# Linyou/Ced-NeRF

Measured on AMD Instinct MI355X. Metric: samples_per_sec (render_image_test, 800x800 D-NeRF lego-shaped synthetic), higher is better.
Workload: dtype f32 (MLP GEMMs: split-fp16 MFMA, 22-bit operands, fp32 accumulate)

## Files before the change

ced_nerf_amd/_lib.py:

```python
from __future__ import annotations

import ctypes as C
import os
import subprocess
from typing import List, Optional

_PKG = os.path.dirname(os.path.abspath(__file__))
_ROOT = os.path.dirname(_PKG)
LIB_PATH = os.environ.get("CED_NERF_LIB", os.path.join(_PKG, "libcednerf_hip.so"))
SOURCES = ["runtime.hip", "march.hip", "composite.hip", "field.hip", "field_half.hip", "field_mixed.hip", "field_move.hip", "field_jacobian.hip", "frame.hip", "occgrid.hip",
           "raygen.hip", "wgrad.hip", "pixels.hip", "accel.hip", "linear.hip", "mlp.hip", "train_glue.hip", "losses.hip",
           "metrics.hip", "train_batch.hip", "importance.hip", "bake.hip", "mesh.hip"]
MLP_F32, MLP_F16X2, MLP_F16, MLP_F32_HEAD16X2 = 0, 1, 2, 3
MLP_PRECISIONS = {"f32": MLP_F32, "f16x2": MLP_F16X2, "f16": MLP_F16, "f32+h16x2": MLP_F32_HEAD16X2}
HIPCC_FLAGS = ["--offload-arch=gfx950", "-O3", "-ffp-contract=off", "-fno-slp-vectorize", "-fPIC", "-shared", "-std=c++17"]
PER_SOURCE_FLAGS = {"field_half.hip": ["-mllvm", "-amdgpu-sched-strategy=max-memory-clause"]}
MAX_LEVELS = 16


class HashDesc(C.Structure):
    _fields_ = [
        ("n_levels", C.c_int32), ("table_dtype", C.c_int32), ("temporal", C.c_int32), ("reserved", C.c_int32),
        ("scale", C.c_float * MAX_LEVELS), ("res", C.c_uint32 * MAX_LEVELS), ("offset", C.c_uint32 * MAX_LEVELS),
        ("size", C.c_uint32 * MAX_LEVELS), ("hashed", C.c_uint32 * MAX_LEVELS),
        ("table", C.c_void_p), ("total_entries", C.c_uint64),
    ]


class FieldDesc(C.Structure):
    _fields_ = [
        ("aabb", C.c_float * 6), ("moving_step", C.c_float), ("use_div_offsets", C.c_int32),
        ("time_mode", C.c_int32), ("mlp_precision", C.c_int32), ("max_workgroups", C.c_int32),
        ("packed_weights", C.c_void_p), ("packed_floats", C.c_uint64),
        ("hash", HashDesc),
    ]


class FrameTrace(C.Structure):
    _fields_ = [
        ("capacity", C.c_int32), ("n_iters", C.c_int32),
        ("field_begin", C.POINTER(C.c_void_p)), ("field_end", C.POINTER(C.c_void_p)),
        ("iter_alive", C.POINTER(C.c_int64)), ("iter_n_samples", C.POINTER(C.c_int64)),
        ("iter_samples", C.POINTER(C.c_int64)), ("field_stamps", C.c_void_p),
    ]


EXCHANGE_FN = C.CFUNCTYPE(C.c_int, C.c_void_p, C.c_void_p, C.c_int32, C.c_int32, C.c_void_p)


class ShardExchange(C.Structure):
    _fields_ = [
        ("global_rays_per_frame", C.c_int64), ("local_rays", C.c_void_p), ("counts", C.c_void_p),
        ("reduce", EXCHANGE_FN), ("user", C.c_void_p),
    ]


_vp, _i64, _i32, _f = C.c_void_p, C.c_int64, C.c_int32, C.c_float

PROTOTYPES = {
    "ced_version": (C.c_int, []),
    "ced_last_error_string": (C.c_char_p, []),
    "ced_set_option": (C.c_int, [C.c_char_p, C.c_int]),
    "ced_packed_weight_floats": (_i64, [C.c_int, C.c_int]),
    "ced_pack_field_weights": (C.c_int, [C.c_int, C.c_int] + [_vp] * 10),
    "ced_packed_weight_words": (_i64, [C.c_int, C.c_int, C.c_int]),
    "ced_pack_field_weights_half": (C.c_int, [C.c_int, C.c_int, C.c_int] + [_vp] * 10),
    "ced_pack_field_weights_half_for": (C.c_int, [C.c_int] * 5 + [_vp] * 10),
    "ced_pack_field_weights_mixed": (C.c_int, [C.c_int, C.c_int] + [_vp] * 10),
    "ced_ray_aabb_intersect": (C.c_int, [_i64, _vp, _vp, _i32, _vp, _f, _f, _f, _vp, _vp, _vp, _vp]),
    "ced_sort_intersections": (C.c_int, [_i64, _i32, _vp, _vp, _vp, _vp, _vp]),
    "ced_traverse_grids": (C.c_int, [_i64, _vp, _vp, _vp, _i32, _i32, _vp, _vp, _vp, _f, _f, _i32, _vp, _vp, _vp, _vp,
                                     _i32, _vp, _vp, _vp, _vp, _vp, _vp, _vp, _vp]),
    "ced_host_skip_march": (_f, [_f, _f, _f, _f]),
    "ced_occupancy_accel_bytes": (_i64, [_i32, _i32]),
    "ced_build_occupancy_accel": (C.c_int, [_vp, _i32, _i32, _vp, _i64, _vp]),
    "ced_host_build_occupancy_accel": (C.c_int, [_vp, _i32, _i32, _vp]),
    "ced_host_count_steps": (_i32, [C.POINTER(C.c_float), _f, _f, _i32, C.POINTER(C.c_float)]),
    "ced_host_march_frame": (C.c_int, [_i64, _vp, _vp, _vp, _i32, _i32, _vp, _vp, _f, _f, _f, _i32, _vp, _vp, _vp, _vp, _i32, _i32,
                                       _i32, _vp, _vp, _vp, _vp]),
    "ced_hash_encode": (C.c_int, [C.POINTER(HashDesc), _i64, _vp, _vp, _vp, _vp]),
    "ced_hash_encode_backward": (C.c_int, [C.POINTER(HashDesc), _i64, _vp, _vp, _vp, _vp, _i32, _vp]),
    "ced_hash_encode_backward_temporal": (C.c_int, [C.POINTER(HashDesc), _i64, _vp, _vp, _vp, _vp, _vp]),
    "ced_field_forward": (C.c_int, [C.POINTER(FieldDesc), _i64, _vp, _vp, _vp, _vp, _vp, _vp, _vp]),
    "ced_field_forward_rays": (C.c_int, [C.POINTER(FieldDesc), _i64, _vp, _vp, _vp, _vp, _vp, _vp, _vp, _i32, _i32,
                                         _vp, _vp, _vp]),
    "ced_field_move": (C.c_int, [C.POINTER(FieldDesc), _i64, _vp, _vp, _vp, _vp, _vp, _vp, _vp]),
    "ced_field_move_rays": (C.c_int, [C.POINTER(FieldDesc), _i64, _vp, _vp, _vp, _vp, _vp, _vp, _vp, _i32, _vp, _vp, _vp]),
    "ced_field_move_inverse": (C.c_int, [C.POINTER(FieldDesc), _i64, _vp, _vp, _vp, _i32, _f, _vp, _vp, _vp, _vp]),
    "ced_field_track": (C.c_int, [C.POINTER(FieldDesc), _i64, _i64, _vp, _vp, _vp, _i32, _f, _vp, _vp, _vp, _vp]),
    "ced_field_move_jacobian": (C.c_int, [C.POINTER(FieldDesc), _i64, _vp, _vp, _vp, _vp, _vp]),
    "ced_field_move_inverse_newton": (C.c_int, [C.POINTER(FieldDesc), _i64, _vp, _vp, _vp, _i32, _f, _vp, _vp, _vp, _vp]),
    "ced_field_track_newton": (C.c_int, [C.POINTER(FieldDesc), _i64, _i64, _vp, _vp, _vp, _i32, _f, _vp, _vp, _vp, _vp]),
    "ced_field_rgb": (C.c_int, [C.POINTER(FieldDesc), _i64, _vp, _vp, _i32, _vp, _vp]),
    "ced_field_rgb_bcast": (C.c_int, [C.POINTER(FieldDesc), _i64, _i32, _vp, _vp, _i32, _vp, _vp]),
    "ced_bake_workspace_bytes": (_i64, [_i64]),
    "ced_bake_candidates": (C.c_int, [_i32, C.POINTER(C.c_float), _f, _i64, _i64, _vp, _vp, _i32, _i32, _i64, _vp, _vp, _vp,
                                      _vp, _i64, _vp]),
    "ced_bake_select": (C.c_int, [_i64, _vp, _vp, _vp, _vp, _f, _i64, _vp, _vp, _vp, _vp, _vp, _vp, _i64, _vp]),
    "ced_mesh_workspace_bytes": (_i64, [_i32]),
    "ced_mesh_vertices": (C.c_int, [_i32, C.POINTER(C.c_float), _f, _vp, _f, _i64, _vp, _vp, _vp, _vp, _vp, _i64, _vp]),
    "ced_mesh_faces": (C.c_int, [_i32, _vp, _f, _vp, _i64, _i64, _vp, _vp, _vp, _i64, _vp]),
    "ced_render_weights": (C.c_int, [_i64, _vp, _vp, _vp, _vp, _vp, _vp, _vp, _vp, _vp]),
    "ced_accumulate_along_rays": (C.c_int, [_i64, _vp, _vp, _vp, _i32, _vp, _vp]),
    "ced_reduce_along_rays": (C.c_int, [_i64, _vp, _vp, _i32, _vp, _i32, _i64, _i32, _vp, _vp, _vp]),
    "ced_visibility_mask": (C.c_int, [_i64, _vp, _vp, _vp, _vp, _f, _f, _vp, _vp]),
    "ced_composite_prefix": (C.c_int, [_i64, _vp, _vp, _vp, _vp, _vp, _vp, _vp, _vp, _vp]),
    "ced_composite_backward": (C.c_int, [_i64, _vp, _vp, _vp, _vp, _vp, _vp, _vp, _vp, _vp, _vp, _vp]),
    "ced_distortion_workspace_bytes": (_i64, [_i64, _i64, _i32]),
    "ced_distortion_loss": (C.c_int, [_i64, _i64] + [_vp] * 10),
    "ced_distortion_loss_density": (C.c_int, [_i64, _i64] + [_vp] * 10),
    "ced_ssim_workspace_bytes": (_i64, [_i64, _i64, _i64, _i64, _i32, _i32]),
    "ced_ssim": (C.c_int, [_i64, _i64, _i64, _i64, _vp, C.POINTER(_i64), _vp, C.POINTER(_i64), C.c_double, C.c_double,
                           C.c_double, _i32, C.POINTER(C.c_float), _i32, C.POINTER(C.c_float), _i32, _vp, _vp, _vp, _vp,
                           _vp, _vp]),
    "ced_frame_to_rgb8": (C.c_int, [_i32, _i32, _vp, _i32, _vp, _vp]),
    "ced_depth_to_u8": (C.c_int, [_i32, _i32, _vp, _i32, _vp, _vp, _vp]),
    "ced_scatter_pixels": (C.c_int, [_i64, _vp, _i32, _vp, _i32, _vp, _i32, _vp, _i64, _vp, _vp, _vp, _vp, _i32, _i32, _vp]),
    "ced_linear": (C.c_int, [_i64, _vp, _i32, _vp, _i32, _i32, _i32, _i32, _i32, _vp, _vp, _vp]),
    "ced_weight_grad_workspace_bytes": (_i64, [_i64, _i32, _i32]),
    "ced_weight_grad": (C.c_int, [_i64, _vp, _i32, _vp, _i32, _vp, _vp, _i64, _vp]),
    "ced_composite_step": (C.c_int, [_i64, _vp, _vp, _vp, _vp, _vp, _vp, _vp, _vp, _f, _i32, _vp, _vp, _vp]),
    "ced_composite_test": (C.c_int, [_i64, _vp, _vp, _vp, _vp, _vp, _vp, _f, _f, _vp, _vp, _vp, _vp]),
    "ced_finalize_pixels": (C.c_int, [_i64, _vp, _vp, _vp, _vp, _vp]),
    "ced_occ_cell_points": (C.c_int, [_i64, _vp, _vp, _i32, C.POINTER(C.c_float), _vp, _vp]),
    "ced_occ_ema_update": (C.c_int, [_i64, _vp, _vp, _f, _f, _vp, _vp]),
    "ced_generate_rays_pinhole": (C.c_int, [_i32, _i32, _f, _f, _f, _f, C.POINTER(C.c_float), _i32, _vp, _vp, _vp, _vp]),
    "ced_generate_rays_hypercam": (C.c_int, [_i32, _i32, C.POINTER(C.c_float), C.POINTER(C.c_float), _f, _f, _f, _f, _f,
                                             C.POINTER(C.c_float), C.POINTER(C.c_float), _vp, _vp, _vp]),
    "ced_sample_training_batch": (C.c_int, [_i32] * 5 + [_vp] * 3 + [_i64, C.c_uint64, _i64, _i32, _i32] + [_vp] * 7),
    "ced_importance_batch_workspace_bytes": (_i64, [_i64, _i64, _i64]),
    "ced_sample_importance_batch": (C.c_int, [_i32] * 5 + [_vp] * 4 + [_i32, _i64, _i64, C.c_uint64, _i64, _i32] + [_vp] * 8
                                    + [_i64, _vp]),
    "ced_temporal_median_u8": (C.c_int, [_i32] * 4 + [_vp] * 3),
    "ced_isg_weights": (C.c_int, [_i32] * 4 + [_vp, _vp, _f, _vp, _vp]),
    "ced_ist_weights": (C.c_int, [_i32] * 4 + [_vp, _f, _i32, _vp, _vp]),
    "ced_render_image_test_workspace_bytes": (_i64, [_i64, _i32, _i32, _f, _i32]),
    "ced_render_image_test": (C.c_int, [C.POINTER(FieldDesc), _i64, _vp, _vp, _vp, _i32, _i32, _vp, _vp, _f, _f, _f, _f, _f,
                                        _i32, _vp, _i32, _vp, _vp, _vp, _vp, _vp, _i64, _vp, C.POINTER(_i64),
                                        C.POINTER(FrameTrace), _vp, _vp]),
    "ced_render_frames_test_workspace_bytes": (_i64, [_i32, _i64, _i32, _i32, _f, _i32]),
    "ced_render_frames_test": (C.c_int, [C.POINTER(FieldDesc), _i32, _i64, _vp, _vp, _vp, _i32, _i32, _vp, _vp, _f, _f, _f, _f,
                                         _f, _i32, _vp, _vp, _vp, _vp, _vp, _vp, _i64, _vp, C.POINTER(_i64),
                                         C.POINTER(FrameTrace), _vp, _vp]),
    "ced_render_frames_test_sharded_workspace_bytes": (_i64, [_i32, _i64, _i64, _i32, _i32, _f, _i32]),
    "ced_render_frames_test_iterations": (_i32, [_f, _i32]),
    "ced_render_frames_test_host_bytes": (_i64, [_f, _i32]),
    "ced_render_frames_test_sharded": (C.c_int, [C.POINTER(FieldDesc), _i32, _i64, _vp, _vp, _vp, _i32, _i32, _vp, _vp, _f, _f, _f,
                                                 _f, _f, _i32, _vp, _vp, _vp, _vp, _vp, _vp, _i64, _vp, C.POINTER(_i64),
                                                 C.POINTER(FrameTrace), _vp, _vp, C.POINTER(ShardExchange)]),
    "ced_wall_clock_khz": (_i64, []),
    "ced_mlp_chain": (C.c_int, [_i64, _i32, _i32, _vp, C.POINTER(_i32), C.POINTER(_vp), C.POINTER(_vp), C.POINTER(_vp), _i32, _vp]),
    "ced_march_all": (C.c_int, [_i64, _vp, _vp, _vp, _i32, _i32, _vp, _vp, _vp, _f, _f, _f, _vp, _vp, _vp, _i32, _vp, _vp, _vp,
                                _vp, _i64, _vp, _vp]),
    "ced_render_image_workspace_bytes": (_i64, [_i64, _i64]),
    "ced_render_image": (C.c_int, [C.POINTER(FieldDesc), _i64, _vp, _vp, _i64, _vp, _vp, _vp, _f, _f, _vp, _i32, _vp, _vp, _vp,
                                   _vp, _vp, _vp, _i64, _vp, C.POINTER(_i64), _vp, _vp]),
    "ced_mlp_backward_dw_workspace_bytes": (_i64, [_i64, _i32, C.POINTER(_i32)]),
    "ced_mlp_backward_dw": (C.c_int, [_i64, _i32, _vp, C.POINTER(_i32), C.POINTER(_vp), C.POINTER(_vp), _vp, _vp, _vp, _i64, _vp]),
    "ced_train_inputs": (C.c_int, [_i64] + [_vp] * 13),
    "ced_train_warp": (C.c_int, [_i64, _vp, _vp, _i32, _i32, _f, C.POINTER(C.c_float), _vp, _vp, _vp, _vp]),
    "ced_train_warp_backward": (C.c_int, [_i64, _vp, _vp, _i32, _i32, _f, C.POINTER(C.c_float), _vp, _vp, _vp, _vp]),
    "ced_train_head_in": (C.c_int, [_i64] + [_vp] * 6),
    "ced_train_head_in_backward": (C.c_int, [_i64] + [_vp] * 6),
    "ced_render_image_gather": (C.c_int, [_i64, _i64, _i64, _vp, _i64, _vp, _i64, _vp, _vp, _vp, _vp, _vp, _vp, _vp, _vp, _vp]),
}


def _includes(path: str, seen=None) -> List[str]:
    import re
    seen = set() if seen is None else seen
    if path in seen or not os.path.exists(path):
        return []
    seen.add(path)
    out = [path]
    for inc in re.findall(r'^\s*#\s*include\s+"([^"]+)"', open(path).read(), flags=re.M):
        out += _includes(os.path.normpath(os.path.join(os.path.dirname(path), inc)), seen)
    return out


def build(force: bool = False, verbose: bool = False, extra_flags: Optional[List[str]] = None) -> str:
    from concurrent.futures import ThreadPoolExecutor
    srcs = [os.path.join(_PKG, "csrc", s) for s in SOURCES]
    hipcc = os.environ.get("HIPCC", "hipcc")
    flags = [f for f in HIPCC_FLAGS if f != "-shared"] + list(extra_flags or [])
    obj_dir = os.path.join(_ROOT, "build", "obj")
    os.makedirs(obj_dir, exist_ok=True)
    stamp = os.path.join(obj_dir, "flags.txt")
    flag_text = " ".join([hipcc] + flags + [f"{k}:{' '.join(v)}" for k, v in sorted(PER_SOURCE_FLAGS.items())])
    if not os.path.exists(stamp) or open(stamp).read() != flag_text:
        force = True
    jobs, objs = [], []
    for src in srcs:
        obj = os.path.join(obj_dir, os.path.basename(src) + ".o")
        objs.append(obj)
        deps = _includes(src)
        if force or not os.path.exists(obj) or any(os.path.getmtime(obj) < os.path.getmtime(d) for d in deps):
            jobs.append([hipcc] + flags + PER_SOURCE_FLAGS.get(os.path.basename(src), []) + ["-c", src, "-o", obj])
    if not jobs and os.path.exists(LIB_PATH) and all(os.path.getmtime(LIB_PATH) >= os.path.getmtime(o) for o in objs):
        return LIB_PATH

    def run(cmd):
        if verbose:
            print(" ".join(cmd), flush=True)
        subprocess.check_call(cmd)

    workers = max(1, min(len(jobs), int(os.environ.get("CED_BUILD_JOBS", str(min(os.cpu_count() or 1, 8))))))
    if jobs:
        with ThreadPoolExecutor(max_workers=workers) as pool:
            list(pool.map(run, jobs))
    run([hipcc, "--offload-arch=gfx950", "-shared", "-fPIC", "-o", LIB_PATH] + objs)
    from . import _k32_gate
    _, bad = _k32_gate.check(LIB_PATH)
    if bad:
        os.remove(LIB_PATH)
        raise RuntimeError("K = 32 residency gate failed (ced_nerf_amd/_k32_gate.py): "
                           + "; ".join(f"{k}: {v}" for k, v in sorted(bad.items())))
    with open(stamp, "w") as f:
        f.write(flag_text)
    return LIB_PATH


_lib: Optional[C.CDLL] = None


def lib() -> C.CDLL:
    global _lib
    if _lib is None:
        if not os.path.exists(LIB_PATH):
            raise RuntimeError(
                f"{LIB_PATH} not found: build the HIP extension first (python -c 'import __graft_entry__ as g; "
                "g.build()'); ced_nerf_amd has no CPU fallback")
        handle = C.CDLL(LIB_PATH)
        for name, (res, args) in PROTOTYPES.items():
            fn = getattr(handle, name)
            fn.restype = res
            fn.argtypes = args
        _lib = handle
        for item in filter(None, os.environ.get("CED_OPTIONS", "").split(",")):
# ... 18 lines not shown
```

ced_nerf_amd/csrc/field.hip:

```cpp
#include <atomic>
#include <cstring>

#include "ced_common.hpp"
#include "field_args.hpp"
#include "field_device.hpp"
#include "field_kernel.hpp"

namespace ced {


struct HashArgs {
    int64_t n;
    const float *x, *t;
    float *out;
    int n_levels, table_dtype, temporal;
    const void *table;
    float scale[CED_MAX_LEVELS];
    uint32_t res[CED_MAX_LEVELS], offset[CED_MAX_LEVELS], size[CED_MAX_LEVELS], hashed[CED_MAX_LEVELS];
};

template <bool F16, bool TEMPORAL>
__global__ __launch_bounds__(256) void hash_encode_kernel(HashArgs A)
{
    const int64_t i = (int64_t)blockIdx.x * blockDim.x + threadIdx.x;
// ... 276 lines not shown
    }
    A.level_mode = 0;
    for (int i = 0; i < 4; ++i) {
        int n_hashed = 0;
        bool pairs = !A.temporal;
        for (int g = 0; g < 4; ++g) {
            const int l = 4 * i + g;
            n_hashed += d->hash.hashed[l] ? 1 : 0;
            pairs = pairs && l + 1 < d->hash.n_levels &&
                    (uint64_t)d->hash.offset[l] + d->hash.size[l] < d->hash.total_entries;
        }
        A.level_mode |= (n_hashed == 0 ? (pairs ? 3 : 1) : (n_hashed == 4 ? 2 : 0)) << (2 * i);
    }
    CED_REQUIRE(d->hash.total_entries * (uint64_t)((A.table_dtype ? 4 : 8) * (A.temporal ? 4 : 1)) < (1ull << 32),
                "field_forward: hash table larger than 4 GiB");
    CED_REQUIRE(d->max_workgroups >= 0 && d->max_workgroups <= 65536, "field_forward: max_workgroups=%d", d->max_workgroups);
    A.max_blocks = d->max_workgroups;
    A.spread_tiles = g_field_spread_tiles;
    if (d->mlp_precision == CED_MLP_F32_HEAD16X2) return launch_field_mixed(A, d->time_mode, stream);
    if (d->mlp_precision != CED_MLP_F32) {
        return launch_field_half(A, d->time_mode, d->mlp_precision, stream);
    }
    switch ((d->time_mode ? 1 : 0) | (A.table_dtype ? 2 : 0) | (A.temporal ? 4 : 0)) {
    case 0: launch_field_grid<2, 1024>(field_kernel<false, false, false, 2, 1024>, A, stream); break;
    case 1: launch_field_grid<2, 1024>(field_kernel<true, false, false, 2, 1024>, A, stream); break;
    case 2: launch_field_grid<2, 1024>(field_kernel<false, true, false, 2, 1024>, A, stream); break;
    case 3: launch_field_grid<2, 1024>(field_kernel<true, true, false, 2, 1024>, A, stream); break;
    case 4: launch_field_grid<2, 512>(field_kernel<false, false, true, 2, 512>, A, stream); break;
    case 5: launch_field_grid<2, 512>(field_kernel<true, false, true, 2, 512>, A, stream); break;
    case 6: launch_field_grid<2, 512>(field_kernel<false, true, true, 2, 512>, A, stream); break;
    default: launch_field_grid<2, 512>(field_kernel<true, true, true, 2, 512>, A, stream); break;
    }
    return check_launch("field_forward");
}

}

extern "C" int ced_set_option(const char *key, int value)
{
    CED_REQUIRE(key != nullptr, "set_option: null key");
    if (strcmp(key, "field_spread_tiles") == 0) {
        CED_REQUIRE(value >= 0 && value <= 2, "set_option: field_spread_tiles must be 0, 1 or 2 (field_tile_range)");
        ced::g_field_spread_tiles = value;
        return CED_OK;
    }
    if (strcmp(key, "march_two_pass") == 0) {
        CED_REQUIRE(value >= -1 && value <= 1, "set_option: march_two_pass must be -1 (automatic), 0 or 1");
        ced::g_march_two_pass = value;
        return CED_OK;
    }
    if (strcmp(key, "hash_grad_blocks") == 0) {
        CED_REQUIRE(value >= 0 && value <= (1 << 20), "set_option: hash_grad_blocks must be 0 (no cap) .. 2^20");
        ced::g_hash_grad_blocks = value;
        return CED_OK;
    }
    ced::set_error("set_option: unknown key '%s'", key);
    return CED_E_INVALID;
}

extern "C" int64_t ced_packed_weight_floats(int use_div_offsets, int time_mode)
{
    (void)use_div_offsets;
    return time_mode ? ced::Blob<true>::TOTAL : ced::Blob<false>::TOTAL;
}

extern "C" int ced_pack_field_weights(int use_div_offsets, int time_mode, const float *m_w0, const float *m_w1,
                                      const float *m_w2, const float *m_w3, const float *b_w0, const float *b_w1,
                                      const float *h_w0, const float *h_w1, const float *h_w2, float *out)
{
    CED_REQUIRE(m_w0 && m_w1 && m_w2 && m_w3 && b_w0 && b_w1 && h_w0 && h_w1 && h_w2 && out,
                "pack_field_weights: null pointer");
    CED_REQUIRE(time_mode >= 0 && time_mode <= 2, "pack_field_weights: time_mode=%d", time_mode);
    const bool te = time_mode != 0;
    const int64_t total = ced_packed_weight_floats(use_div_offsets, time_mode);
    for (int64_t i = 0; i < total; ++i) out[i] = 0.0f;
    struct L { const float *w; int n_out, n_in, nb, ks, off; int placement; };
    const int base_in = te ? 41 : 32;
    const int n_mo = use_div_offsets ? 6 : 3;
    const int ksb0 = te ? 11 : 8;
    int offs[9];
    if (te) {
        using B = ced::Blob<true>;
        int o[9] = { B::M0, B::M1, B::M2, B::M3, B::B0, B::B1, B::H0, B::H1, B::H2 };
        for (int i = 0; i < 9; ++i) offs[i] = o[i];
    } else {
        using B = ced::Blob<false>;
        int o[9] = { B::M0, B::M1, B::M2, B::M3, B::B0, B::B1, B::H0, B::H1, B::H2 };
        for (int i = 0; i < 9; ++i) offs[i] = o[i];
    }
    const L layers[9] = {
        { m_w0, 64, 32, 4, 8, offs[0], 1 },      { m_w1, 64, 64, 4, 16, offs[1], 1 },
        { m_w2, 64, 64, 4, 16, offs[2], 1 },     { m_w3, n_mo, 64, 1, 16, offs[3], 0 },
        { b_w0, 64, base_in, 4, ksb0, offs[4], 1 }, { b_w1, 16, 64, 1, 16, offs[5], 2 },
        { h_w0, 64, 19, 4, 5, offs[6], 1 },      { h_w1, 64, 64, 4, 16, offs[7], 1 },
        { h_w2, 3, 64, 1, 16, offs[8], 3 },
    };
    for (const L &l : layers) {
        const int ks4 = ced::ks4_of(l.ks);
        for (int p = 0; p < l.nb * 16; ++p) {
            int neuron = p;
            if (l.placement == 1) neuron = (p & ~15) | ((p & 3) << 2) | ((p >> 2) & 3);
            else if (l.placement == 2) neuron = ced::base_out_neuron(p);
            else if (l.placement == 3) neuron = (p & 3) ? l.n_out : (p >> 2);
            if (neuron >= l.n_out) continue;
            for (int k = 0; k < l.ks * 4; ++k) {
                if (k >= l.n_in) continue;
                const int S = k / 4, kk = k % 4;
                const int lane = kk * 16 + (p % 16);
                const int64_t idx = l.off + (((int64_t)(p / 16) * ks4 + S / 4) * 64 + lane) * 4 + (S % 4);
                out[idx] = l.w[(int64_t)neuron * l.n_in + k];
            }
        }
    }
    return CED_OK;
}

extern "C" int ced_field_forward(const ced_field_desc *desc, int64_t n, const float *positions, const float *t,
                                 const float *directions, float *rgb, float *sigma, float *geo, void *stream)
{
    CED_REQUIRE(desc != nullptr, "field_forward: null descriptor");
    CED_REQUIRE(n >= 0, "field_forward: n < 0");
    if (n == 0) return CED_OK;
    CED_REQUIRE(positions && t && sigma, "field_forward: null positions/t/sigma");
    CED_REQUIRE((directions != nullptr) == (rgb != nullptr), "field_forward: directions and rgb go together");
    ced::FieldArgs A{};
    A.n = n;
    A.pos = positions; A.t = t; A.dir = directions;
    A.rays_mode = 0; A.t_per_ray = 0; A.want_rgb = rgb ? 1 : 0;
    A.rgb = rgb; A.sigma = sigma; A.geo = geo;
    return ced::launch_field(desc, A, stream);
}

extern "C" int ced_field_forward_rays(const ced_field_desc *desc, int64_t n, const int64_t *n_dev,
                                      const float *rays_o, const float *rays_d, const int64_t *ray_indices, const float *t_starts, const float *t_ends,
                                      const float *timestamps, int32_t t_per_ray, int32_t want_rgb, float *rgb,
                                      float *sigma, void *stream)
{
    CED_REQUIRE(desc != nullptr, "field_forward_rays: null descriptor");
    CED_REQUIRE(n >= 0, "field_forward_rays: n < 0");
    if (n == 0) return CED_OK;
    CED_REQUIRE(rays_o && rays_d && ray_indices && t_starts && t_ends && timestamps && sigma,
                "field_forward_rays: null pointer");
    CED_REQUIRE(!want_rgb || rgb, "field_forward_rays: want_rgb without an rgb buffer");
    ced::FieldArgs A{};
    A.n = n;
    A.n_dev = n_dev;
    A.rays_o = rays_o; A.rays_d = rays_d; A.ray_idx = ray_indices;
    A.t0 = t_starts; A.t1 = t_ends; A.timestamps = timestamps;
    A.rays_mode = 1; A.t_per_ray = t_per_ray ? 1 : 0; A.want_rgb = want_rgb ? 1 : 0;
    A.rgb = rgb; A.sigma = sigma; A.geo = nullptr;
    return ced::launch_field(desc, A, stream);
}

extern "C" int ced_hash_encode(const ced_hash_desc *desc, int64_t n, const float *x, const float *t, float *out,
                               void *stream)
{
    int rc = ced::validate_hash(desc, "hash_encode");
    if (rc) return rc;
    CED_REQUIRE(n >= 0, "hash_encode: n < 0");
    if (n == 0) return CED_OK;
    CED_REQUIRE(x && out, "hash_encode: null pointer");
    ced::HashArgs A{};
    A.n = n; A.x = x; A.t = t; A.out = out;
    A.n_levels = desc->n_levels; A.table_dtype = desc->table_dtype; A.temporal = desc->temporal ? 1 : 0;
    A.table = desc->table;
    for (int l = 0; l < CED_MAX_LEVELS; ++l) {
        A.scale[l] = desc->scale[l]; A.res[l] = desc->res[l]; A.offset[l] = desc->offset[l];
        A.size[l] = desc->size[l]; A.hashed[l] = desc->hashed[l];
    }
    const dim3 grid((unsigned)((n + 255) / 256)), block(256);
    const int sel = (A.table_dtype ? 1 : 0) | (A.temporal ? 2 : 0);
    switch (sel) {
    case 0: hipLaunchKernelGGL((ced::hash_encode_kernel<false, false>), grid, block, 0, (hipStream_t)stream, A); break;
    case 1: hipLaunchKernelGGL((ced::hash_encode_kernel<true, false>), grid, block, 0, (hipStream_t)stream, A); break;
    case 2: hipLaunchKernelGGL((ced::hash_encode_kernel<false, true>), grid, block, 0, (hipStream_t)stream, A); break;
    default: hipLaunchKernelGGL((ced::hash_encode_kernel<true, true>), grid, block, 0, (hipStream_t)stream, A); break;
    }
    return ced::check_launch("hash_encode");
}

extern "C" int ced_hash_encode_backward(const ced_hash_desc *desc, int64_t n, const float *x, const float *dy,
                                        float *grad_table, float *dx, int32_t dx_scaled, void *stream)
{
    int rc = ced::validate_hash(desc, "hash_encode_backward");
    if (rc) return rc;
    CED_REQUIRE(n >= 0, "hash_encode_backward: n < 0");
    CED_REQUIRE(!desc->temporal, "hash_encode_backward: the temporal table has no backward yet");
    CED_REQUIRE(desc->n_levels <= 16, "hash_encode_backward: n_levels > 16");
    if (n == 0) return CED_OK;
    CED_REQUIRE(x && dy && (grad_table || dx), "hash_encode_backward: null pointer");
    ced::HashBwdArgs A{};
    A.n = n; A.x = x; A.dy = dy; A.grad_table = grad_table; A.dx = dx;
    A.n_levels = desc->n_levels; A.table_dtype = desc->table_dtype; A.table = desc->table;
    A.dx_scaled = dx_scaled ? 1 : 0;
    for (int l = 0; l < CED_MAX_LEVELS; ++l) {
        A.scale[l] = desc->scale[l]; A.res[l] = desc->res[l]; A.offset[l] = desc->offset[l];
        A.size[l] = desc->size[l]; A.hashed[l] = desc->hashed[l];
    }
    const dim3 block(256);
    if (grad_table) {
        int64_t gx = (4 * n + 255) / 256;
        const int cap = ced::g_hash_grad_blocks;
        if (cap > 0 && gx > cap) gx = cap;
        const dim3 grid_t((unsigned)gx, (unsigned)desc->n_levels);
        hipLaunchKernelGGL(ced::hash_table_grad_kernel, grid_t, block, 0, (hipStream_t)stream, A);
    }
    if (dx) {
        const dim3 grid_x((unsigned)((n * 16 + 255) / 256));
        if (A.table_dtype) hipLaunchKernelGGL(ced::hash_backward_kernel<true>, grid_x, block, 0, (hipStream_t)stream, A);
        else hipLaunchKernelGGL(ced::hash_backward_kernel<false>, grid_x, block, 0, (hipStream_t)stream, A);
    }
    return ced::check_launch("hash_encode_backward");
}

extern "C" int ced_hash_encode_backward_temporal(const ced_hash_desc *desc, int64_t n, const float *x, const float *t,
                                                 const float *dy, float *grad_table, void *stream)
{
    int rc = ced::validate_hash(desc, "hash_encode_backward_temporal");
    if (rc) return rc;
    CED_REQUIRE(n >= 0, "hash_encode_backward_temporal: n < 0");
    CED_REQUIRE(desc->temporal, "hash_encode_backward_temporal: the table is not temporal (use ced_hash_encode_backward)");
    CED_REQUIRE(desc->n_levels <= 16, "hash_encode_backward_temporal: n_levels > 16");
    CED_REQUIRE(desc->total_entries * 8ull < (1ull << 32), "hash_encode_backward_temporal: table too large for 32-bit slots");
    if (n == 0) return CED_OK;
    CED_REQUIRE(x && t && dy && grad_table, "hash_encode_backward_temporal: null pointer");
    ced::HashBwdArgs A{};
    A.n = n; A.x = x; A.t = t; A.dy = dy; A.grad_table = grad_table;
    A.n_levels = desc->n_levels; A.table_dtype = desc->table_dtype; A.table = desc->table;
    for (int l = 0; l < CED_MAX_LEVELS; ++l) {
        A.scale[l] = desc->scale[l]; A.res[l] = desc->res[l]; A.offset[l] = desc->offset[l];
        A.size[l] = desc->size[l]; A.hashed[l] = desc->hashed[l];
    }
    int64_t gx = (4 * n + 255) / 256;
    const int cap = ced::g_hash_grad_blocks;
    if (cap > 0 && gx > cap) gx = cap;
    hipLaunchKernelGGL(ced::hash_table_grad_temporal_kernel, dim3((unsigned)gx, (unsigned)desc->n_levels), dim3(256), 0,
                       (hipStream_t)stream, A);
    return ced::check_launch("hash_encode_backward_temporal");
}
```

ced_nerf_amd/csrc/field_args.hpp:

```cpp
#pragma once
#include <hip/hip_runtime.h>
#include <atomic>
#include <cstdint>

#include "../../include/cednerf_hip.h"

namespace ced {

struct FieldArgs {
    int64_t n;
    const int64_t *n_dev;
    unsigned long long *stamp;
    const int64_t *base_dev;
    const float *pos, *t, *dir;
    const float *rays_o, *rays_d;
    const int64_t *ray_idx;
    const int32_t *ray_idx32;
    const float *t0, *t1, *timestamps;
    int rays_mode, t_per_ray, want_rgb;
    float *rgb, *sigma, *geo;
    float aabb[6];
    float moving_step;
    int use_div, time_mode;
    const void *weights;
    int table_dtype, temporal;
    int spread_tiles;
    int level_mode;
    int max_blocks;
    const void *table;
    float scale[CED_MAX_LEVELS];
    uint32_t res[CED_MAX_LEVELS], offset[CED_MAX_LEVELS], size[CED_MAX_LEVELS], hashed[CED_MAX_LEVELS];
};

extern std::atomic<int> g_march_two_pass;
extern std::atomic<int> g_field_spread_tiles;
constexpr int kFieldBlocksDefault = 256;

template <int NT, int THREADS, typename Kernel>
void launch_field_grid(Kernel kernel, const FieldArgs &A, void *stream)
{
    const int64_t n_tiles = (A.n + 16 * NT - 1) / (16 * NT);
    constexpr int waves = THREADS / 64;
    int64_t blocks = A.spread_tiles ? (n_tiles + 3) / 4 : (n_tiles + waves - 1) / waves;
    const int cap = A.max_blocks > 0 ? A.max_blocks : kFieldBlocksDefault;
    if (blocks > cap) blocks = cap;
    hipLaunchKernelGGL(kernel, dim3((unsigned)blocks), dim3(THREADS), 0, (hipStream_t)stream, A);
}

int launch_field(const ced_field_desc *d, FieldArgs &A, void *stream);
int launch_field_half(FieldArgs &A, int time_mode, int precision, void *stream);
int launch_field_mixed(FieldArgs &A, int time_mode, void *stream);

}
```

ced_nerf_amd/csrc/field_half.hip:

```cpp
#include <cstring>

#include "ced_common.hpp"
#include "field_args.hpp"
#include "field_device.hpp"
#include "field_half_device.hpp"

namespace ced {

template <bool TE, bool F16, bool TEMPORAL, bool SPLIT, int NT, int THREADS>
__global__ __launch_bounds__(THREADS) void field_half_kernel(FieldArgs A)
{
    constexpr int WAVES = THREADS / kWave;
    constexpr bool K32 = half_kernel_k32(TE, TEMPORAL, SPLIT, THREADS);
    static_assert(!K32 || (WAVES & (WAVES - 1)) == 0, "field_tile_seq needs a power-of-two wave count");
    constexpr int TILE = 16 * NT;
    using BL = HalfBlob<TE>;
    constexpr int PLANE = BL::FRAGS * kFragHalves;
    constexpr int WHALVES = PLANE * (SPLIT ? 2 : 1);
    __shared__ __attribute__((aligned(16))) _Float16 lds[WHALVES + 16 * CED_MAX_LEVELS];
    __shared__ int next_elem;
    const int tid = threadIdx.x;
    const int lane = tid & 63;
    const int wave = __builtin_amdgcn_readfirstlane(tid >> 6);
    const int g = lane >> 4, c = lane & 15;

    int64_t n_eff = A.n;
    if (A.n_dev) {
        const int64_t nd = *A.n_dev;
        n_eff = nd < n_eff ? nd : n_eff;
    }
    const int64_t sbase = A.base_dev ? *A.base_dev : 0;
    const int64_t n_tiles = (n_eff + TILE - 1) / TILE;
    TileRange tiles;
    TileSeq seq;
    if constexpr (K32) {
        if (!field_tile_seq(A.spread_tiles, n_tiles, WAVES, seq)) return;
        tiles.first = field_tile_at(seq, wave);
        tiles.end = seq.end;
        tiles.stride = 0;
        if (tid == 0) next_elem = WAVES;
    } else {
        if (!field_tile_range(A.spread_tiles, n_tiles, WAVES, wave, tiles)) return;
    }
    if (A.stamp && tid == 0) atomicMin(A.stamp, (unsigned long long)wall_clock64());

    {
        const f4 *src = reinterpret_cast<const f4 *>(A.weights);
        f4 *dst = reinterpret_cast<f4 *>(lds);
        for (int i = tid; i < WHALVES / 8; i += THREADS) dst[i] = src[i];
        if (tid < CED_MAX_LEVELS) {
            uint32_t *lt = reinterpret_cast<uint32_t *>(lds + WHALVES);
            const LevelConst L = make_level(A.scale[tid], A.res[tid], A.offset[tid], A.size[tid], A.hashed[tid],
                                            EntryBytes<F16, TEMPORAL>::value);
            store_level(lt + tid * 8, L);
        }
    }
    __syncthreads();

    const float extent[3] = { A.aabb[3] - A.aabb[0], A.aabb[4] - A.aabb[1], A.aabb[5] - A.aabb[2] };

    auto next_tile = [&](int64_t tile) -> int64_t {
        if constexpr (K32) {
            int i = 0;
            if (lane == 0) i = atomicAdd(&next_elem, 1);
            return field_tile_at(seq, __builtin_amdgcn_readfirstlane(i));
        } else {
            return tile + tiles.stride;
        }
    };
    for (int64_t tile = tiles.first; tile < tiles.end; tile = next_tile(tile)) {
        int lds_off = 0;
        asm volatile("" : "+v"(lds_off));
        const _Float16 *const whi = lds + lds_off;
        const _Float16 *const wlo = whi + PLANE;
        const int64_t tile_base = tile * TILE;
        const int64_t left = n_eff - tile_base;
        const int in_tile = left < TILE ? (int)left : TILE;
        int sofs[NT];
        int64_t ridx[NT];
        float px[NT][3], tq[NT];
        bool any_used = !A.rays_mode;
#pragma unroll
        for (int j = 0; j < NT; ++j) {
            sofs[j] = 16 * j + c < in_tile ? 16 * j + c : in_tile - 1;
            const int64_t s = tile_base + sofs[j];
            if (A.rays_mode) {
                const int64_t r_in = A.ray_idx32 ? (int64_t)A.ray_idx32[sbase + s] : A.ray_idx[sbase + s];
                const bool used = r_in >= 0;
                const int64_t r = used ? r_in : 0;
                any_used = any_used || used;
                ridx[j] = r;
                const float tm2 = used ? A.t0[sbase + s] + A.t1[sbase + s] : 0.0f;
#pragma unroll
                for (int a = 0; a < 3; ++a) px[j][a] = A.rays_o[3 * r + a] + (A.rays_d[3 * r + a] * tm2) / 2.0f;
                tq[j] = A.t_per_ray ? A.timestamps[r] : A.timestamps[0];
            } else {
                ridx[j] = s;
#pragma unroll
                for (int a = 0; a < 3; ++a) px[j][a] = A.pos[3 * s + a];
                tq[j] = A.t[s];
            }
        }

        if (__ballot(any_used) == 0ull) continue;

        h8 Bh[NT][2], Bl[NT][2];
        f4 D[NT][4];

#pragma unroll
        for (int j = 0; j < NT; ++j) {
            float v = tq[j];
            v = (g == 0) ? px[j][0] : v;
            v = (g == 1) ? px[j][1] : v;
            v = (g == 2) ? px[j][2] : v;
            float f[8];
#pragma unroll
            for (int e = 0; e < 8; ++e) f[e] = det_sinpi_phase(v * (float)(1 << (e >> 1)), e & 1);
            to_half8<SPLIT>(f, Bh[j][0], Bl[j][0]);
        }
        mlp_layer_h<1, 4, NT, SPLIT>(whi + BL::M0 * kFragHalves, wlo + BL::M0 * kFragHalves, lane, Bh, Bl, D);
        to_operand_h<NT, SPLIT>(D, Bh, Bl);
        mlp_layer_h<2, 4, NT, SPLIT, K32>(whi + BL::M1 * kFragHalves, wlo + BL::M1 * kFragHalves, lane, Bh, Bl, D);
        to_operand_h<NT, SPLIT>(D, Bh, Bl);
        mlp_layer_h<2, 4, NT, SPLIT, K32>(whi + BL::M2 * kFragHalves, wlo + BL::M2 * kFragHalves, lane, Bh, Bl, D);
        to_operand_h<NT, SPLIT>(D, Bh, Bl);
        mlp_layer_h<2, 1, NT, SPLIT, K32>(whi + BL::M3 * kFragHalves, wlo + BL::M3 * kFragHalves, lane, Bh, Bl, D);

        float xn[NT][3], mnorm[NT];
        bool sel[NT];
#pragma unroll
        for (int j = 0; j < NT; ++j) {
            float mv[3];
            bool inside = true;
#pragma unroll
            for (int a = 0; a < 3; ++a) {
                const float off = __shfl(D[j][0][a], c, 64);
                float m = off * A.moving_step;
                if (A.use_div) {
                    constexpr int kFineReg[3] = { 3, 0, 1 };
                    const float fine = __shfl(D[j][0][kFineReg[a]], (a == 0) ? c : 16 + c, 64);
                    const float e = det_expf(2.0f * fine);
                    const float th = 1.0f - 2.0f / (e + 1.0f);
                    m = m + th * A.moving_step;
                }
                mv[a] = m;
                const float xm = px[j][a] + m;
                const float x = (xm - A.aabb[a]) / extent[a];
                inside = inside && (x > 0.0f && x < 1.0f);
                xn[j][a] = __builtin_fminf(__builtin_fmaxf(x, 0.0f), 1.0f);
            }
            sel[j] = inside;
            mnorm[j] = TE ? __builtin_sqrtf((mv[0] * mv[0] + mv[1] * mv[1]) + mv[2] * mv[2]) : 0.0f;
        }

        float R[NT][8];
        int k_lo[NT];
        float t_frac[NT];
#pragma unroll
        for (int j = 0; j < NT; ++j) {
            k_lo[j] = 0;
            t_frac[j] = 0.0f;
            if constexpr (TEMPORAL) temporal_keyframe(tq[j], k_lo[j], t_frac[j]);
        }
        const uint32_t *const ltab = reinterpret_cast<const uint32_t *>(whi + WHALVES);
#pragma unroll
        for (int i = 0; i < 4; ++i) {
            const LevelConst L = load_level(ltab + (4 * i + g) * 8);
            const int mode = (A.level_mode >> (2 * i)) & 3;
            if (mode == 1) {
#pragma unroll
                for (int j = 0; j < NT; ++j)
                    hash_level<F16, TEMPORAL, 1>(L, A.table, xn[j], k_lo[j], t_frac[j], R[j][2 * i], R[j][2 * i + 1]);
            } else if (mode == 2) {
#pragma unroll
                for (int j = 0; j < NT; ++j)
                    hash_level<F16, TEMPORAL, 2>(L, A.table, xn[j], k_lo[j], t_frac[j], R[j][2 * i], R[j][2 * i + 1]);
            } else if (mode == 3) {
#pragma unroll
                for (int j = 0; j < NT; ++j)
                    hash_level<F16, TEMPORAL, 3>(L, A.table, xn[j], k_lo[j], t_frac[j], R[j][2 * i], R[j][2 * i + 1]);
            } else {
#pragma unroll
                for (int j = 0; j < NT; ++j)
                    hash_level<F16, TEMPORAL, 0>(L, A.table, xn[j], k_lo[j], t_frac[j], R[j][2 * i], R[j][2 * i + 1]);
            }
        }
#pragma unroll
        for (int j = 0; j < NT; ++j) {
#pragma unroll
            for (int e = 0; e < 8; ++e) R[j][e] = __builtin_amdgcn_fmed3f(R[j][e], -kHalfMax, kHalfMax);
            to_half8<SPLIT>(R[j], Bh[j][0], Bl[j][0]);
            if constexpr (TE) {
                float tf[8];
#pragma unroll
                for (int e = 0; e < 8; ++e) tf[e] = (e < 3) ? time_feature(4 * e + g, A.time_mode, tq[j], mnorm[j]) : 0.0f;
                to_half8<SPLIT>(tf, Bh[j][1], Bl[j][1]);
            }
        }

        mlp_layer_h<BL::KS_B0, 4, NT, SPLIT>(whi + BL::B0 * kFragHalves, wlo + BL::B0 * kFragHalves, lane, Bh, Bl, D);
        to_operand_h<NT, SPLIT>(D, Bh, Bl);
        mlp_layer_h<2, 1, NT, SPLIT, K32>(whi + BL::B1 * kFragHalves, wlo + BL::B1 * kFragHalves, lane, Bh, Bl, D);

#pragma unroll
        for (int j = 0; j < NT; ++j) {
            const bool stored = 16 * j + c < in_tile;
            const int64_t s = tile_base + (16 * j + c);
            float sg = det_expf(D[j][0][3] - 1.0f);
            sg = sel[j] ? sg : 0.0f;
            if (g == 3 && stored) A.sigma[sbase + s] = sg;
            if (A.geo && stored) {
#pragma unroll
                for (int r = 0; r < 4; ++r)
                    if (4 * g + r < 15) A.geo[s * 15 + 4 * g + r] = D[j][0][r];
            }
        }

        if (A.want_rgb) {
#pragma unroll
            for (int j = 0; j < NT; ++j) {
                float dv[3];
#pragma unroll
                for (int a = 0; a < 3; ++a)
                    dv[a] = A.rays_mode ? A.rays_d[3 * ridx[j] + a] : A.dir[3 * (tile_base + sofs[j]) + a];
                const float nrm = __builtin_sqrtf((dv[0] * dv[0] + dv[1] * dv[1]) + dv[2] * dv[2]);
                const float comp = (g == 1) ? dv[1] : (g == 2) ? dv[2] : dv[0];
                const float u = (comp / nrm + 1.0f) / 2.0f;
                const float vv = u * 2.0f - 1.0f;
                const float coef = (g == 2) ? 0.48860251190291987f : -0.48860251190291987f;
                const float sh = (g == 0) ? 0.28209479177387814f : coef * vv;
                float hin[8];
                hin[0] = sh;
#pragma unroll
                for (int r = 0; r < 4; ++r) hin[1 + r] = __builtin_amdgcn_fmed3f(D[j][0][r], -kHalfMax, kHalfMax);
                hin[4] = (g == 3) ? 0.0f : hin[4];
                hin[5] = hin[6] = hin[7] = 0.0f;
                to_half8<SPLIT>(hin, Bh[j][0], Bl[j][0]);
            }
            mlp_layer_h<1, 4, NT, SPLIT>(whi + BL::H0 * kFragHalves, wlo + BL::H0 * kFragHalves, lane, Bh, Bl, D);
            to_operand_h<NT, SPLIT>(D, Bh, Bl);
            mlp_layer_h<2, 4, NT, SPLIT, K32>(whi + BL::H1 * kFragHalves, wlo + BL::H1 * kFragHalves, lane, Bh, Bl, D);
            to_operand_h<NT, SPLIT>(D, Bh, Bl);
            mlp_layer_h<2, 1, NT, SPLIT, K32>(whi + BL::H2 * kFragHalves, wlo + BL::H2 * kFragHalves, lane, Bh, Bl, D);
#pragma unroll
            for (int j = 0; j < NT; ++j) {
                const int64_t s = tile_base + (16 * j + c);
                const float o1 = 1.0f / (1.0f + det_expf(-D[j][0][0]));
                if (g < 3 && 16 * j + c < in_tile) A.rgb[3 * (sbase + s) + g] = o1;
            }
        }
    }
    if constexpr (K32) {
        __syncthreads();
        asm volatile("" ::: "v127");
    }
    if (A.stamp && lane == 0) atomicMax(A.stamp + 1, (unsigned long long)wall_clock64());
}

void pack_half_layer(const float *w, int n_out, int n_in, int nb, int ks, int frag, int row_map, int col_map,
                     _Float16 *hi, _Float16 *lo)
{
    for (int p = 0; p < nb * 16; ++p) {
        int neuron = p;
        if (row_map == HALF_ROW_HIDDEN) neuron = half_hidden_neuron(p);
        else if (row_map == HALF_ROW_HIDDEN_K32) neuron = half_hidden_neuron_k32(p);
        else if (row_map == HALF_ROW_BASE_OUT) neuron = half_base_out_neuron(p);
        else if (row_map == HALF_ROW_RGB) neuron = (p % 4 == 0) ? p / 4 : n_out;
        if (neuron >= n_out) continue;
        for (int k = 0; k < ks * 32; ++k) {
            const int g = (k % 32) / 8, e = k % 8;
            int in = k;
            if (col_map == HALF_COL_HASH) {
                if (k < 32) in = 2 * (4 * (e >> 1) + g) + (e & 1);
                else in = (e < 3 && 4 * e + g <= 8) ? 32 + 4 * e + g : -1;
            } else if (col_map == HALF_COL_K32) {
                in = half_hidden_neuron_k32(16 * (2 * (k / 32) + (e >> 2)) + 4 * g + (e & 3));
            } else if (col_map == HALF_COL_HEAD) {
                if (e == 0) in = g;
                else if (e <= 4 && 4 * g + e - 1 < 15) in = 4 + 4 * g + e - 1;
                else in = -1;
            }
            if (in < 0 || in >= n_in) continue;
            const float v = w[(int64_t)neuron * n_in + in];
            const _Float16 h = (_Float16)v;
            const int64_t idx = ((int64_t)(frag + (p / 16) * ks + k / 32) * 64 + 16 * g + (p % 16)) * 8 + e;
            hi[idx] = h;
            if (lo) lo[idx] = (_Float16)(v - (float)h);
        }
    }
}

int launch_field_half(FieldArgs &A, int time_mode, int precision, void *stream)
{
    const int sel = (time_mode ? 1 : 0) | (A.table_dtype ? 2 : 0) | (A.temporal ? 4 : 0);
    if (precision == CED_MLP_F16X2) {
        switch (sel) {
        case 0: launch_field_grid<2, 1024>(field_half_kernel<false, false, false, true, 2, 1024>, A, stream); break;
        case 1: launch_field_grid<2, 768>(field_half_kernel<true, false, false, true, 2, 768>, A, stream); break;
        case 2: launch_field_grid<2, 1024>(field_half_kernel<false, true, false, true, 2, 1024>, A, stream); break;
        case 3: launch_field_grid<2, 768>(field_half_kernel<true, true, false, true, 2, 768>, A, stream); break;
        case 4: launch_field_grid<2, 512>(field_half_kernel<false, false, true, true, 2, 512>, A, stream); break;
        case 5: launch_field_grid<2, 512>(field_half_kernel<true, false, true, true, 2, 512>, A, stream); break;
        case 6: launch_field_grid<2, 512>(field_half_kernel<false, true, true, true, 2, 512>, A, stream); break;
        default: launch_field_grid<2, 512>(field_half_kernel<true, true, true, true, 2, 512>, A, stream); break;
        }
    } else {
        switch (sel) {
        case 0: launch_field_grid<2, 768>(field_half_kernel<false, false, false, false, 2, 768>, A, stream); break;
        case 1: launch_field_grid<2, 768>(field_half_kernel<true, false, false, false, 2, 768>, A, stream); break;
        case 2: launch_field_grid<2, 768>(field_half_kernel<false, true, false, false, 2, 768>, A, stream); break;
        case 3: launch_field_grid<2, 768>(field_half_kernel<true, true, false, false, 2, 768>, A, stream); break;
        case 4: launch_field_grid<2, 512>(field_half_kernel<false, false, true, false, 2, 512>, A, stream); break;
        case 5: launch_field_grid<2, 512>(field_half_kernel<true, false, true, false, 2, 512>, A, stream); break;
        case 6: launch_field_grid<2, 512>(field_half_kernel<false, true, true, false, 2, 512>, A, stream); break;
        default: launch_field_grid<2, 512>(field_half_kernel<true, true, true, false, 2, 512>, A, stream); break;
        }
    }
    return check_launch("field_forward (half-precision MLP)");
}

}

extern "C" int64_t ced_packed_weight_words(int use_div_offsets, int time_mode, int mlp_precision)
{
    if (mlp_precision == CED_MLP_F32 || mlp_precision == CED_MLP_F32_HEAD16X2) return ced_packed_weight_floats(use_div_offsets, time_mode);
    if (mlp_precision != CED_MLP_F16X2 && mlp_precision != CED_MLP_F16) return -1;
    const int64_t frags = time_mode ? ced::HalfBlob<true>::FRAGS : ced::HalfBlob<false>::FRAGS;
    return frags * (ced::kFragHalves / 2) * (mlp_precision == CED_MLP_F16X2 ? 2 : 1);
}

static int pack_half(int use_div_offsets, int time_mode, int mlp_precision, bool k32, const float *m_w0, const float *m_w1,
                     const float *m_w2, const float *m_w3, const float *b_w0, const float *b_w1, const float *h_w0,
                     const float *h_w1, const float *h_w2, void *out)
{
    CED_REQUIRE(m_w0 && m_w1 && m_w2 && m_w3 && b_w0 && b_w1 && h_w0 && h_w1 && h_w2 && out,
                "pack_field_weights_half: null pointer");
    CED_REQUIRE(time_mode >= 0 && time_mode <= 2, "pack_field_weights_half: time_mode=%d", time_mode);
    CED_REQUIRE(mlp_precision == CED_MLP_F16X2 || mlp_precision == CED_MLP_F16,
                "pack_field_weights_half: mlp_precision=%d (1 = f16x2, 2 = f16)", mlp_precision);
    const bool te = time_mode != 0, split = mlp_precision == CED_MLP_F16X2;
    const int64_t words = ced_packed_weight_words(use_div_offsets, time_mode, mlp_precision);
    memset(out, 0, (size_t)words * 4);
    _Float16 *hi = reinterpret_cast<_Float16 *>(out);
    _Float16 *lo = hi + (te ? ced::HalfBlob<true>::FRAGS : ced::HalfBlob<false>::FRAGS) * ced::kFragHalves;
    using namespace ced;
    struct L { const float *w; int n_out, n_in, nb, ks, frag, row, col; };
    const int base_in = te ? 41 : 32, n_mo = use_div_offsets ? 6 : 3, ksb0 = te ? 2 : 1;
    int fr[9];
    if (te) {
        using B = HalfBlob<true>;
        const int o[9] = { B::M0, B::M1, B::M2, B::M3, B::B0, B::B1, B::H0, B::H1, B::H2 };
        for (int i = 0; i < 9; ++i) fr[i] = o[i];
    } else {
        using B = HalfBlob<false>;
        const int o[9] = { B::M0, B::M1, B::M2, B::M3, B::B0, B::B1, B::H0, B::H1, B::H2 };
        for (int i = 0; i < 9; ++i) fr[i] = o[i];
    }
    const int HR = k32 ? HALF_ROW_HIDDEN_K32 : HALF_ROW_HIDDEN, HC = k32 ? HALF_COL_K32 : HALF_COL_NATURAL;
    const L layers[9] = {
        { m_w0, 64, 32, 4, 1, fr[0], HR, HALF_COL_NATURAL },         { m_w1, 64, 64, 4, 2, fr[1], HR, HC },
        { m_w2, 64, 64, 4, 2, fr[2], HR, HC },                       { m_w3, n_mo, 64, 1, 2, fr[3], HALF_ROW_NATURAL, HC },
        { b_w0, 64, base_in, 4, ksb0, fr[4], HR, HALF_COL_HASH },    { b_w1, 16, 64, 1, 2, fr[5], HALF_ROW_BASE_OUT, HC },
        { h_w0, 64, 19, 4, 1, fr[6], HR, HALF_COL_HEAD },            { h_w1, 64, 64, 4, 2, fr[7], HR, HC },
        { h_w2, 3, 64, 1, 2, fr[8], HALF_ROW_RGB, HC },
    };
    for (const L &l : layers) pack_half_layer(l.w, l.n_out, l.n_in, l.nb, l.ks, l.frag, l.row, l.col, hi, split ? lo : nullptr);
    return CED_OK;
}

extern "C" int ced_pack_field_weights_half(int use_div_offsets, int time_mode, int mlp_precision, const float *m_w0,
                                           const float *m_w1, const float *m_w2, const float *m_w3, const float *b_w0,
                                           const float *b_w1, const float *h_w0, const float *h_w1, const float *h_w2,
                                           void *out)
{
    return pack_half(use_div_offsets, time_mode, mlp_precision, false, m_w0, m_w1, m_w2, m_w3, b_w0, b_w1, h_w0, h_w1,
                     h_w2, out);
}

extern "C" int ced_pack_field_weights_half_for(int use_div_offsets, int time_mode, int mlp_precision, int table_dtype,
                                               int temporal, const float *m_w0, const float *m_w1, const float *m_w2,
                                               const float *m_w3, const float *b_w0, const float *b_w1, const float *h_w0,
                                               const float *h_w1, const float *h_w2, void *out)
{
    CED_REQUIRE(table_dtype == 0 || table_dtype == 1, "pack_field_weights_half_for: table_dtype=%d (0 = fp32, 1 = fp16)",
                table_dtype);
    return pack_half(use_div_offsets, time_mode, mlp_precision, ced::half_layout_k32(time_mode, mlp_precision, temporal),
                     m_w0, m_w1, m_w2, m_w3, b_w0, b_w1, h_w0, h_w1, h_w2, out);
}
```

ced_nerf_amd/csrc/field_kernel.hpp:

```cpp
#pragma once
#include "ced_common.hpp"
#include "field_args.hpp"
#include "field_device.hpp"
#include "field_half_device.hpp"

namespace ced {

struct LayerShape { int nb; int ks; };
__host__ __device__ constexpr int ks4_of(int ks) { return (ks + 3) / 4; }
__host__ __device__ constexpr int layer_floats(int nb, int ks) { return nb * ks4_of(ks) * 256; }

__host__ __device__ constexpr int base_out_neuron(int p)
{
    const int g = p >> 2, r = p & 3;
    return r > 0 ? (4 * r + g - 3) : (g < 3 ? 13 + g : 0);
}

template <bool TE> struct Blob {
    static constexpr int KS_B0 = TE ? 11 : 8;
    static constexpr int M0 = 0;
    static constexpr int M1 = M0 + layer_floats(4, 8);
    static constexpr int M2 = M1 + layer_floats(4, 16);
    static constexpr int M3 = M2 + layer_floats(4, 16);
    static constexpr int B0 = M3 + layer_floats(1, 16);
    static constexpr int B1 = B0 + layer_floats(4, KS_B0);
    static constexpr int H0 = B1 + layer_floats(1, 16);
    static constexpr int H1 = H0 + layer_floats(4, 5);
    static constexpr int H2 = H1 + layer_floats(4, 16);
    static constexpr int TOTAL = H2 + layer_floats(1, 16);
    static constexpr int HEAD_FRAGS = 14;
    static constexpr int HF_H0 = 0, HF_H1 = 4, HF_H2 = 12;
    static_assert(2 * HEAD_FRAGS * kFragHalves * 2 == (TOTAL - H0) * 4, "the fp16 head must fill the fp32 head's region");
};
constexpr int kMaxBlobFloats = Blob<true>::TOTAL;


template <int KS, int NB, int NT>
__device__ __forceinline__ void mlp_layer(const float *__restrict__ wl, int lane, const float (&B)[NT][16],
                                          f4 (&D)[NT][4])
{
    constexpr int KS4 = ks4_of(KS);
    constexpr int G = NB * KS4;
    f4 a = *reinterpret_cast<const f4 *>(wl + lane * 4);
    f4 acc[NT];
#pragma unroll
    for (int grp = 0; grp < G; ++grp) {
        const int nb = grp / KS4, q = grp % KS4;
        if (q == 0) {
#pragma unroll
            for (int j = 0; j < NT; ++j) acc[j] = f4{ 0.0f, 0.0f, 0.0f, 0.0f };
        }
        f4 a_next = a;
        if (grp + 1 < G) a_next = *reinterpret_cast<const f4 *>(wl + ((grp + 1) * 64 + lane) * 4);
#pragma unroll
        for (int s = 0; s < 4; ++s) {
            if (4 * q + s < KS) {
#pragma unroll
                for (int j = 0; j < NT; ++j)
                    acc[j] = __builtin_amdgcn_mfma_f32_16x16x4f32(a[s], B[j][4 * q + s], acc[j], 0, 0, 0);
            }
        }
        if (q == KS4 - 1) {
#pragma unroll
            for (int j = 0; j < NT; ++j) D[j][nb] = acc[j];
        }
        a = a_next;
    }
}

template <int NB, bool RELU, int NT>
__device__ __forceinline__ void to_operand(const f4 (&D)[NT][4], float (&B)[NT][16])
{
#pragma unroll
    for (int j = 0; j < NT; ++j) {
#pragma unroll
        for (int nb = 0; nb < NB; ++nb) {
            float r[4];
#pragma unroll
            for (int q = 0; q < 4; ++q) {
                float v = D[j][nb][q];
                if constexpr (RELU) {
                    const int bits = __float_as_int(v);
                    v = __int_as_float(bits > 0 ? bits : 0);
                }
                r[q] = v;
            }
#pragma unroll
            for (int s = 0; s < 4; ++s) B[j][4 * nb + s] = r[s];
        }
    }
}

template <bool TE, bool F16, bool TEMPORAL, int NT, int THREADS, bool HEAD16 = false>
__global__ __launch_bounds__(THREADS) void field_kernel(FieldArgs A)
{
    constexpr int FIELD_THREADS = THREADS;
    constexpr int FIELD_WAVES = THREADS / kWave;
    constexpr int TILE = 16 * NT;
    using BL = Blob<TE>;
    __shared__ __attribute__((aligned(16))) float lds[BL::TOTAL + 8 * CED_MAX_LEVELS];
    const int tid = threadIdx.x;
    const int lane = tid & 63;
    const int g = lane >> 4, c = lane & 15;

    int64_t n_eff = A.n;
    if (A.n_dev) {
        const int64_t nd = *A.n_dev;
        n_eff = nd < n_eff ? nd : n_eff;
    }
    const int64_t sbase = A.base_dev ? *A.base_dev : 0;
    const int64_t n_tiles = (n_eff + TILE - 1) / TILE;
    TileRange tiles;
    if (!field_tile_range(A.spread_tiles, n_tiles, FIELD_WAVES, threadIdx.x >> 6, tiles)) return;
    if (A.stamp && tid == 0) atomicMin(A.stamp, (unsigned long long)wall_clock64());

    {
        const f4 *src = reinterpret_cast<const f4 *>(A.weights);
        f4 *dst = reinterpret_cast<f4 *>(lds);
        for (int i = tid; i < BL::TOTAL / 4; i += FIELD_THREADS) dst[i] = src[i];
        if (tid < CED_MAX_LEVELS) {
            uint32_t *lt = reinterpret_cast<uint32_t *>(lds + BL::TOTAL);
            const LevelConst L = make_level(A.scale[tid], A.res[tid], A.offset[tid], A.size[tid], A.hashed[tid],
                                            EntryBytes<F16, TEMPORAL>::value);
            store_level(lt + tid * 8, L);
        }
    }
    __syncthreads();

    const float extent[3] = { A.aabb[3] - A.aabb[0], A.aabb[4] - A.aabb[1], A.aabb[5] - A.aabb[2] };
    const bool shared_time = A.rays_mode && !A.t_per_ray;
    float t_feat[2] = { 0.0f, 0.0f };
    if (shared_time) {
        const float t_all = A.timestamps[0];
#pragma unroll
        for (int S = 6; S < 8; ++S) t_feat[S - 6] = det_sinpi_phase(t_all * (float)(1 << (2 * (S & 1) + (g >> 1))), g & 1);
    }

    for (int64_t tile = tiles.first; tile < tiles.end; tile += tiles.stride) {
        int lds_off = 0;
        asm volatile("" : "+v"(lds_off));
        const float *const lw = lds + lds_off;
        int64_t sidx[NT];
        int64_t ridx[NT];
        float px[NT][3], tq[NT];
        bool any_used = !A.rays_mode;
#pragma unroll
        for (int j = 0; j < NT; ++j) {
            int64_t s = tile * TILE + 16 * j + c;
            s = s < n_eff ? s : n_eff - 1;
            sidx[j] = s;
            if (A.rays_mode) {
                const int64_t r_in = A.ray_idx32 ? (int64_t)A.ray_idx32[sbase + s] : A.ray_idx[sbase + s];
                const bool used = r_in >= 0;
                const int64_t r = used ? r_in : 0;
                any_used = any_used || used;
                ridx[j] = r;
                const float tm2 = used ? A.t0[sbase + s] + A.t1[sbase + s] : 0.0f;
#pragma unroll
                for (int a = 0; a < 3; ++a) px[j][a] = A.rays_o[3 * r + a] + (A.rays_d[3 * r + a] * tm2) / 2.0f;
                tq[j] = A.t_per_ray ? A.timestamps[r] : A.timestamps[0];
            } else {
                ridx[j] = s;
#pragma unroll
                for (int a = 0; a < 3; ++a) px[j][a] = A.pos[3 * s + a];
                tq[j] = A.t[s];
            }
        }
        if (__ballot(any_used) == 0ull) continue;

        float B[NT][16];
        f4 D[NT][4];

#pragma unroll
        for (int j = 0; j < NT; ++j) {
            const bool odd = (g & 1) != 0;
            const float sc0 = (float)(1 << (g >> 1)), sc1 = 4.0f * sc0;
            const float vxy = odd ? px[j][1] : px[j][0];
            float p0, p1;
            det_sinpi_both(vxy * sc0, p0, p1);
            auto sw = __builtin_amdgcn_permlane16_swap(__float_as_uint(p0), __float_as_uint(p1), false, false);
            B[j][0] = __uint_as_float(sw[0]); B[j][2] = __uint_as_float(sw[1]);
            det_sinpi_both(vxy * sc1, p0, p1);
            sw = __builtin_amdgcn_permlane16_swap(__float_as_uint(p0), __float_as_uint(p1), false, false);
            B[j][1] = __uint_as_float(sw[0]); B[j][3] = __uint_as_float(sw[1]);
            const float scz = odd ? sc1 : sc0;
            det_sinpi_both(px[j][2] * scz, p0, p1);
            sw = __builtin_amdgcn_permlane16_swap(__float_as_uint(p0), __float_as_uint(p1), false, false);
            B[j][4] = __uint_as_float(sw[0]); B[j][5] = __uint_as_float(sw[1]);
            if (shared_time) {
                B[j][6] = t_feat[0];
                B[j][7] = t_feat[1];
            } else {
                det_sinpi_both(tq[j] * scz, p0, p1);
                sw = __builtin_amdgcn_permlane16_swap(__float_as_uint(p0), __float_as_uint(p1), false, false);
                B[j][6] = __uint_as_float(sw[0]); B[j][7] = __uint_as_float(sw[1]);
            }
        }
        mlp_layer<8, 4, NT>(lw + BL::M0, lane, B, D);
        to_operand<4, true, NT>(D, B);
        mlp_layer<16, 4, NT>(lw + BL::M1, lane, B, D);
        to_operand<4, true, NT>(D, B);
        mlp_layer<16, 4, NT>(lw + BL::M2, lane, B, D);
        to_operand<4, true, NT>(D, B);
        mlp_layer<16, 1, NT>(lw + BL::M3, lane, B, D);

        float xn[NT][3], mnorm[NT];
        bool sel[NT];
#pragma unroll
        for (int j = 0; j < NT; ++j) {
            float mv[3];
            bool inside = true;
#pragma unroll
            for (int a = 0; a < 3; ++a) {
                const float off = __shfl(D[j][0][a], c, 64);
                float m = off * A.moving_step;
                if (A.use_div) {
                    constexpr int kFineReg[3] = { 3, 0, 1 };
                    const float fine = __shfl(D[j][0][kFineReg[a]], (a == 0) ? c : 16 + c, 64);
                    const float e = det_expf(2.0f * fine);
                    const float th = 1.0f - 2.0f / (e + 1.0f);
                    m = m + th * A.moving_step;
                }
                mv[a] = m;
                const float xm = px[j][a] + m;
                const float x = (xm - A.aabb[a]) / extent[a];
                inside = inside && (x > 0.0f && x < 1.0f);
                xn[j][a] = __builtin_fminf(__builtin_fmaxf(x, 0.0f), 1.0f);
            }
            sel[j] = inside;
            mnorm[j] = TE ? __builtin_sqrtf((mv[0] * mv[0] + mv[1] * mv[1]) + mv[2] * mv[2]) : 0.0f;
        }

        float R[NT][8];
        int k_lo[NT];
        float t_frac[NT];
#pragma unroll
        for (int j = 0; j < NT; ++j) {
            k_lo[j] = 0;
            t_frac[j] = 0.0f;
            if constexpr (TEMPORAL) temporal_keyframe(tq[j], k_lo[j], t_frac[j]);
        }
        const uint32_t *const ltab = reinterpret_cast<const uint32_t *>(lw + BL::TOTAL);
#pragma unroll
        for (int i = 0; i < 4; ++i) {
            const LevelConst L = load_level(ltab + (4 * i + 2 * (g & 1) + (g >> 1)) * 8);
            const int mode = (A.level_mode >> (2 * i)) & 3;
            if (mode == 1) {
#pragma unroll
                for (int j = 0; j < NT; ++j)
                    hash_level<F16, TEMPORAL, 1>(L, A.table, xn[j], k_lo[j], t_frac[j], R[j][2 * i], R[j][2 * i + 1]);
            } else if (mode == 2) {
#pragma unroll
                for (int j = 0; j < NT; ++j)
                    hash_level<F16, TEMPORAL, 2>(L, A.table, xn[j], k_lo[j], t_frac[j], R[j][2 * i], R[j][2 * i + 1]);
            } else if (mode == 3) {
#pragma unroll
                for (int j = 0; j < NT; ++j)
                    hash_level<F16, TEMPORAL, 3>(L, A.table, xn[j], k_lo[j], t_frac[j], R[j][2 * i], R[j][2 * i + 1]);
            } else {
#pragma unroll
                for (int j = 0; j < NT; ++j)
                    hash_level<F16, TEMPORAL, 0>(L, A.table, xn[j], k_lo[j], t_frac[j], R[j][2 * i], R[j][2 * i + 1]);
            }
        }
#pragma unroll
        for (int j = 0; j < NT; ++j) {
#pragma unroll
            for (int i = 0; i < 4; ++i) {
                auto sw = __builtin_amdgcn_permlane16_swap(__float_as_uint(R[j][2 * i]), __float_as_uint(R[j][2 * i + 1]), false, false);
                B[j][2 * i] = __uint_as_float(sw[0]);
                B[j][2 * i + 1] = __uint_as_float(sw[1]);
            }
            if (TE) {
#pragma unroll
                for (int S = 8; S < 11; ++S) B[j][S] = time_feature(4 * (S - 8) + g, A.time_mode, tq[j], mnorm[j]);
            }
        }

        mlp_layer<BL::KS_B0, 4, NT>(lw + BL::B0, lane, B, D);
        to_operand<4, true, NT>(D, B);
        mlp_layer<16, 1, NT>(lw + BL::B1, lane, B, D);

#pragma unroll
        for (int j = 0; j < NT; ++j) {
            const int64_t s = tile * TILE + 16 * j + c;
            float sg = det_expf(D[j][0][HEAD16 ? 3 : 0] - 1.0f);
            sg = sel[j] ? sg : 0.0f;
            if (g == 3 && s < n_eff) A.sigma[sbase + s] = sg;
            if (A.geo && s < n_eff) {
#pragma unroll
                for (int r = 0; r < 4; ++r) {
                    const int nidx = HEAD16 ? half_base_out_neuron(4 * g + r) : base_out_neuron(4 * g + r);
                    if (nidx >= 1) A.geo[s * 15 + nidx - 1] = D[j][0][r];
                }
            }
        }

        if constexpr (HEAD16) {
            if (A.want_rgb) {
                const _Float16 *const hw = reinterpret_cast<const _Float16 *>(lw + BL::H0);
                const _Float16 *const hwl = hw + BL::HEAD_FRAGS * kFragHalves;
                h8 Bh[NT][2], Bl[NT][2];
#pragma unroll
                for (int j = 0; j < NT; ++j) {
                    float dv[3];
#pragma unroll
                    for (int a = 0; a < 3; ++a)
                        dv[a] = A.rays_mode ? A.rays_d[3 * ridx[j] + a] : A.dir[3 * sidx[j] + a];
                    const float nrm = __builtin_sqrtf((dv[0] * dv[0] + dv[1] * dv[1]) + dv[2] * dv[2]);
                    const float comp = (g == 1) ? dv[1] : (g == 2) ? dv[2] : dv[0];
                    const float u = (comp / nrm + 1.0f) / 2.0f;
                    const float vv = u * 2.0f - 1.0f;
                    const float coef = (g == 2) ? 0.48860251190291987f : -0.48860251190291987f;
                    float hin[8];
                    hin[0] = (g == 0) ? 0.28209479177387814f : coef * vv;
#pragma unroll
                    for (int r = 0; r < 4; ++r) hin[1 + r] = __builtin_amdgcn_fmed3f(D[j][0][r], -kHalfMax, kHalfMax);
                    hin[4] = (g == 3) ? 0.0f : hin[4];
                    hin[5] = hin[6] = hin[7] = 0.0f;
                    to_half8<true>(hin, Bh[j][0], Bl[j][0]);
                }
                mlp_layer_h<1, 4, NT, true>(hw + BL::HF_H0 * kFragHalves, hwl + BL::HF_H0 * kFragHalves, lane, Bh, Bl, D);
                to_operand_h<NT, true>(D, Bh, Bl);
                mlp_layer_h<2, 4, NT, true>(hw + BL::HF_H1 * kFragHalves, hwl + BL::HF_H1 * kFragHalves, lane, Bh, Bl, D);
                to_operand_h<NT, true>(D, Bh, Bl);
                mlp_layer_h<2, 1, NT, true>(hw + BL::HF_H2 * kFragHalves, hwl + BL::HF_H2 * kFragHalves, lane, Bh, Bl, D);
#pragma unroll
                for (int j = 0; j < NT; ++j) {
                    const float o1 = 1.0f / (1.0f + det_expf(-D[j][0][0]));
                    int lane_now = (int)threadIdx.x;
                    asm volatile("" : "+v"(lane_now));
                    const int g_now = (lane_now >> 4) & 3;
                    const int64_t s_now = tile * TILE + 16 * j + (lane_now & 15);
                    if (g_now < 3 && s_now < n_eff) A.rgb[3 * (sbase + s_now) + g_now] = o1;
                }
            }
            continue;
        }

        if (A.want_rgb) {
#pragma unroll
            for (int j = 0; j < NT; ++j) {
                const float geo_tail = (g == 3) ? 0.0f : D[j][0][0];
                float dv[3];
#pragma unroll
                for (int a = 0; a < 3; ++a)
                    dv[a] = A.rays_mode ? A.rays_d[3 * ridx[j] + a] : A.dir[3 * sidx[j] + a];
                const float nrm = __builtin_sqrtf((dv[0] * dv[0] + dv[1] * dv[1]) + dv[2] * dv[2]);
                const float comp = (g == 1) ? dv[1] : (g == 2) ? dv[2] : dv[0];
                const float u = (comp / nrm + 1.0f) / 2.0f;
                const float vv = u * 2.0f - 1.0f;
                const float coef = (g == 2) ? 0.48860251190291987f : -0.48860251190291987f;
                B[j][0] = (g == 0) ? 0.28209479177387814f : coef * vv;
                B[j][1] = D[j][0][1];
                B[j][2] = D[j][0][2];
                B[j][3] = D[j][0][3];
                B[j][4] = geo_tail;
            }
            mlp_layer<5, 4, NT>(lw + BL::H0, lane, B, D);
            to_operand<4, true, NT>(D, B);
            mlp_layer<16, 4, NT>(lw + BL::H1, lane, B, D);
            to_operand<4, true, NT>(D, B);
            mlp_layer<16, 1, NT>(lw + BL::H2, lane, B, D);
#pragma unroll
            for (int j = 0; j < NT; ++j) {
                const int64_t s = tile * TILE + 16 * j + c;
                const float o1 = 1.0f / (1.0f + det_expf(-D[j][0][0]));
                int lane_now = (int)threadIdx.x;
                asm volatile("" : "+v"(lane_now));
                const int g_now = (lane_now >> 4) & 3;
                const int64_t s_now = tile * TILE + 16 * j + (lane_now & 15);
                if (g_now < 3 && s_now < n_eff) A.rgb[3 * (sbase + s_now) + g_now] = o1;
            }
        }
    }
    if (A.stamp && lane == 0) atomicMax(A.stamp + 1, (unsigned long long)wall_clock64());
}

}
```

ced_nerf_amd/csrc/frame.hip:

```cpp
#include <atomic>
#include <cfloat>
#include <chrono>
#include <vector>

#include "ced_common.hpp"
#include "field_args.hpp"
#include "march_accel.hpp"

#ifdef CED_MARCH_DIAG
__device__ unsigned long long g_march_diag[8][3];
__device__ __forceinline__ unsigned long long (*ced_diag_acc())[8][3]
{
    __shared__ unsigned long long acc[16][8][3];
    return acc;
}
__device__ __forceinline__ unsigned long long *ced_diag_state()
{
    __shared__ unsigned long long st[16][2];
    return &st[0][0];
}
__device__ void ced_diag_tick(int phase)
{
    const unsigned long long m = __ballot(1);
    const int wave = threadIdx.x >> 6;
// ... 140 lines not shown
                                                         const float *__restrict__ rays_d, int m,
                                                         const float *__restrict__ aabbs, float near_plane,
                                                         float *__restrict__ t_sorted, uint8_t *__restrict__ t_indices,
                                                         uint8_t *__restrict__ hits, float *__restrict__ near_planes,
                                                         float *__restrict__ rgb,
                                                         float *__restrict__ opacity, float *__restrict__ depth)
{
    int64_t r = (int64_t)blockIdx.x * blockDim.x + threadIdx.x;
    if (r >= n_rays) return;
    const float o[3] = { rays_o[3 * r], rays_o[3 * r + 1], rays_o[3 * r + 2] };
    const float inv_d[3] = { 1.0f / rays_d[3 * r], 1.0f / rays_d[3 * r + 1], 1.0f / rays_d[3 * r + 2] };
    float ev[2 * kMaxGrids];
    int id[2 * kMaxGrids];
    for (int a = 0; a < m; ++a) {
        float t0 = __builtin_inff(), t1 = __builtin_inff();
        bool hit = slab_test(o, inv_d, aabbs + 6 * a, t0, t1);
        if (!hit) { t0 = __builtin_inff(); t1 = __builtin_inff(); }
        hits[r * m + a] = hit ? 1 : 0;
        ev[a] = t0; id[a] = a;
        ev[m + a] = t1; id[m + a] = m + a;
    }
    if (m > 1) {
        for (int i = 1; i < 2 * m; ++i) {
            float v = ev[i];
            int k = id[i], j = i - 1;
            while (j >= 0 && ev[j] > v) { ev[j + 1] = ev[j]; id[j + 1] = id[j]; --j; }
            ev[j + 1] = v; id[j + 1] = k;
        }
    }
    for (int i = 0; i < 2 * m; ++i) {
        t_sorted[r * 2 * m + i] = ev[i];
        t_indices[r * 2 * m + i] = (uint8_t)id[i];
    }
    near_planes[r] = near_plane;
    rgb[3 * r] = 0.0f; rgb[3 * r + 1] = 0.0f; rgb[3 * r + 2] = 0.0f;
    opacity[r] = 0.0f;
    depth[r] = 0.0f;
}

__global__ __launch_bounds__(256) void frame_prep_single_kernel(int64_t n_rays, float near_plane, float *__restrict__ near_planes,
                                                                float *__restrict__ rgb, float *__restrict__ opacity,
                                                                float *__restrict__ depth)
{
    int64_t r = (int64_t)blockIdx.x * blockDim.x + threadIdx.x;
    if (r >= n_rays) return;
    near_planes[r] = near_plane;
    rgb[3 * r] = 0.0f; rgb[3 * r + 1] = 0.0f; rgb[3 * r + 2] = 0.0f;
    opacity[r] = 0.0f;
    depth[r] = 0.0f;
}

struct ScheduleArgs {
    IterPlan *plans;
    int it, n_frames, rays_per_frame, min_samples, max_samples;
    long long *host;
    long long seq;
    const int32_t *local_rays;
    const int64_t *xcounts;
    int64_t global_rays;
    long long *host_iter;
};

__device__ __forceinline__ void make_next_plan(const ScheduleArgs &S)
{
    const int f = threadIdx.x & 63;
    IterPlan &N = S.plans[S.it + 1];
    int local = 0, used = 0;
    long long global = 0;
    if (f < S.n_frames) {
        if (S.it < 0) {
            local = S.local_rays ? S.local_rays[f] : S.rays_per_frame;
            global = S.global_rays > 0 ? S.global_rays : local;
        } else {
            const IterPlan &P = S.plans[S.it];
            const unsigned long long nx = __hip_atomic_load(&P.next[f], __ATOMIC_RELAXED, __HIP_MEMORY_SCOPE_AGENT);
            const bool finished = P.last[f] || P.gcount[f] == 0;
            local = (finished || P.count[f] == 0) ? 0 : (int)(nx & 0xffffffffull);
            global = finished ? 0 : (S.xcounts ? S.xcounts[(int64_t)S.it * S.n_frames + f] : local);
            used = P.used[f];
        }
    }
    int count = 0, gcount = 0, limit = 0, last = 0;
    if (global > 0 && used < S.max_samples) {
        const long long n_total = S.global_rays > 0 ? S.global_rays : S.rays_per_frame;
        const long long q = n_total / global;
        limit = q < 64 ? (int)q : 64;
        if (limit < S.min_samples) limit = S.min_samples;
        used += limit;
        last = used >= S.max_samples ? 1 : 0;
        count = local;
        gcount = (int)(global < 0x7fffffffll ? global : 0x7fffffffll);
    }
    const int padded = (count + kSlotAlign - 1) & ~(kSlotAlign - 1);
    int incl = padded;
#pragma unroll
    for (int off = 1; off < 64; off <<= 1) {
        const int v = __shfl_up(incl, off, 64);
        if (f >= off) incl += v;
    }
    long long alive_here = count, alive_all = gcount;
#pragma unroll
    for (int off = 32; off >= 1; off >>= 1) {
        alive_here += __shfl_xor(alive_here, off, 64);
        alive_all += __shfl_xor(alive_all, off, 64);
    }
    const int total_slots = __shfl(incl, 63, 64);
    N.count[f] = count; N.gcount[f] = gcount; N.limit[f] = limit; N.last[f] = last; N.used[f] = used;
    N.slot_base[f] = incl - padded; N.samp_bound[f] = count * limit;
    N.next[f] = 0;
    if (f == 0) {
        N.total_slots = total_slots;
        N.sample_base = S.it < 0 ? 0 : S.plans[S.it].sample_base + S.plans[S.it].total_samples;
        N.total_samples = 0;
        N.n_cand = 0;
        N.cursor = 0;
        N.done = alive_all == 0 ? 1 : 0;
        S.host[0] = alive_here;
        S.host[1] = N.done;
        if (S.host_iter) {
            S.host_iter[3 * (S.it + 1)] = alive_here;
            S.host_iter[3 * (S.it + 1) + 1] = N.done;
        }
        __threadfence_system();
        __hip_atomic_store(&S.host[2], S.seq, __ATOMIC_RELEASE, __HIP_MEMORY_SCOPE_SYSTEM);
        if (S.host_iter) __hip_atomic_store(&S.host_iter[3 * (S.it + 1) + 2], S.seq, __ATOMIC_RELEASE, __HIP_MEMORY_SCOPE_SYSTEM);
    }
}

__global__ void frame_init_kernel(ScheduleArgs S, float *__restrict__ lattice_dev, unsigned long long *stamps = nullptr,
                                  int n_stamps = 0)
{
    for (int i = threadIdx.x; i < n_stamps; i += blockDim.x) {
        stamps[2 * i] = ~0ull;
        stamps[2 * i + 1] = 0ull;
    }
    if (lattice_dev) {
        const float *src = reinterpret_cast<const float *>(S.host + kHostLatticeWord);
        for (int i = threadIdx.x; i < 256; i += blockDim.x) lattice_dev[i] = src[i];
    }
    if (threadIdx.x < 64) make_next_plan(S);
}

struct MarchArgs {
    const float *rays_o, *rays_d;
    GridSpec grid;
    AccelSpec accel;
    float *near_planes;
    float far_plane;
    const int32_t *alive;
    int n_frames, rays_per_frame;
    const float *t_sorted;
    const uint8_t *t_indices;
    const uint8_t *hits;
    float *t_starts, *t_ends;
    int32_t *ray_idx;
    int32_t *packed;
    int32_t *cand;
};

constexpr int kMaxRuns = 4;

struct SampleRuns {
    float t[kMaxRuns] = {};
    int n[kMaxRuns] = {};
    int count = 0;
    float prev_end = 0.0f;

    __device__ __forceinline__ void record(int i, float t0, float t1)
    {
        const bool fresh = i == 0 || t0 != prev_end;
        if (fresh) ++count;
        prev_end = t1;
#pragma unroll
        for (int k = 0; k < kMaxRuns; ++k) {
            const bool here = count == k + 1;
            t[k] = (here && fresh) ? t0 : t[k];
            n[k] += here ? 1 : 0;
        }
    }
    __device__ __forceinline__ bool replayable(const GridSpec &grid) const { return count <= kMaxRuns && grid.step_size > 0.0f; }
    template <class Store>
    __device__ __forceinline__ void replay(const GridSpec &grid, Store store) const
    {
        int pos = 0;
#pragma unroll
        for (int k = 0; k < kMaxRuns; ++k) {
            float ts = t[k];
            for (int j = 0; j < n[k]; ++j) {
                const float te = ts + calc_dt(ts, grid.cone_angle, grid.step_size, 1e10f);
                store(pos++, ts, te);
                ts = te;
            }
        }
    }
};

constexpr int kCullThreads = 256;
static_assert(kSlotAlign % kCullThreads == 0, "a culling workgroup's slots belong to one frame");
template <bool SINGLE>
__global__ __launch_bounds__(kCullThreads) void march_cull_kernel(MarchArgs A, IterPlan *__restrict__ plan)
{
    const IterPlan &P = *plan;
    const int64_t total = P.total_slots;
    const int m = SINGLE ? 1 : A.grid.n_grids, res = A.grid.res;
    for (int64_t s0 = (int64_t)blockIdx.x * kCullThreads; s0 < total; s0 += (int64_t)gridDim.x * kCullThreads) {
        const int f = frame_of_slot(P, A.n_frames, s0);
        if (f < 0) continue;
        const int64_t idx = s0 + threadIdx.x - P.slot_base[f];
        const bool active = idx < P.count[f];
        const int64_t r = (int64_t)f * A.rays_per_frame + (active ? idx : 0);
        bool cand = false;
        if (active) {
            float o[3], d[3];
#pragma unroll
            for (int a = 0; a < 3; ++a) { o[a] = A.rays_o[3 * r + a]; d[a] = A.rays_d[3 * r + a]; }
            const float near = A.near_planes[r];
            if constexpr (SINGLE) {
                const float inv_d[3] = { 1.0f / d[0], 1.0f / d[1], 1.0f / d[2] };
                float seg_a, seg_b;
                if (slab_test(o, inv_d, A.grid.aabbs, seg_a, seg_b)) {
                    const float t0 = fmaxf(seg_a, near), t1 = fminf(seg_b, A.far_plane);
                    float t_stop, cells;
                    if (t0 < t1) cand = !coarse_advance(A.accel, 0, res, A.grid.aabbs, o, d, t0, t1, t_stop, cells);
                }
            } else {
                const float *ts_row = A.t_sorted + r * 2 * m;
                const uint8_t *ti_row = A.t_indices + r * 2 * m;
                const uint8_t *hit_row = A.hits + r * m;
                for (int i = 0; i < 2 * m - 1 && !cand; ++i) {
                    const int ti = ti_row[i];
                    int lvl = (int)(ti % m);
                    if (!hit_row[lvl]) continue;
                    if (!(ti < m)) {
                        const int tn = ti_row[i + 1];
                        if (tn < m) continue;
                        lvl = (int)(tn % m);
                        if (!hit_row[lvl]) continue;
                    }
                    const float t0 = fmaxf(ts_row[i], near), t1 = fminf(ts_row[i + 1], A.far_plane);
                    if (t0 >= t1) continue;
                    float t_stop, cells;
                    cand = !coarse_advance(A.accel, lvl, res, A.grid.aabbs + 6 * lvl, o, d, t0, t1, t_stop, cells);
                }
            }
            if (!cand) { A.packed[2 * r] = 0; A.packed[2 * r + 1] = 0; }
        }
        const int slot = workgroup_append<kCullThreads / 64, 0>(
            cand, nullptr, [&](int run, const int *) { return run > 0 ? atomicAdd(&plan->n_cand, run) : 0; });
        if (cand) A.cand[slot] = (int32_t)r;
        __syncthreads();
    }
}

constexpr int kCandLanes = 64;
template <bool SINGLE, bool CAND, bool FIRST>
__global__ __launch_bounds__(kMarchThreads, (SINGLE && !CAND) ? 4 : 3) void march_frame_kernel(MarchArgs A, IterPlan *__restrict__ plan)
{
    static_assert(!CAND || FIRST, "the candidate list belongs to the first iteration");
    constexpr int kWaves = kMarchThreads / 64;
    constexpr int kPerGroup = CAND ? kWaves * kCandLanes : kMarchThreads;
    const IterPlan &P = *plan;
    const int64_t total = CAND ? (int64_t)P.n_cand : (int64_t)P.total_slots;
    const int lane = threadIdx.x & 63, wave = threadIdx.x >> 6;
    for (int64_t s0 = (int64_t)blockIdx.x * kPerGroup; s0 < total; s0 += (int64_t)gridDim.x * kPerGroup) {
        int f = 0;
        bool active;
        int64_t r = 0;
        if constexpr (CAND) {
            const int64_t slot = s0 + wave * kCandLanes + lane;
            active = lane < kCandLanes && slot < total;
            if (active) { r = A.cand[slot]; f = (int)(r / A.rays_per_frame); }
        } else {
            f = frame_of_slot(P, A.n_frames, s0);
            if (f < 0) continue;
            const int64_t idx = s0 + threadIdx.x - P.slot_base[f];
            active = idx < P.count[f];
            const int64_t first = (int64_t)f * A.rays_per_frame;
            r = active ? (A.alive ? (int64_t)A.alive[first + idx] : first + idx) : 0;
        }
        const int limit = P.limit[f];
        GridSpec grid = A.grid;
        grid.limit = limit;
        const int m = grid.n_grids;
        float o[3] = { 0.0f, 0.0f, 0.0f }, d[3] = { 0.0f, 0.0f, 1.0f };
        float near = 0.0f, t_term = 0.0f;
        const auto walk = [&](auto &&emit, float &t_out) {
            return traverse_ray_frame<kFrameLook, SINGLE, FIRST>(
                grid, A.accel, FIRST, o, d, near, A.far_plane,
                SINGLE ? nullptr : A.t_sorted + r * 2 * m, SINGLE ? (const uint8_t *)nullptr : A.t_indices + r * 2 * m,
                SINGLE ? nullptr : A.hits + r * m, emit, t_out);
        };
        SampleRuns runs;
        int n = 0;
        CED_DIAG_TICK(0);
        if (active) {
#pragma unroll
            for (int a = 0; a < 3; ++a) { o[a] = A.rays_o[3 * r + a]; d[a] = A.rays_d[3 * r + a]; }
            near = A.near_planes[r];
            n = walk([&](int i, float t0, float t1) { runs.record(i, t0, t1); }, t_term);
            A.near_planes[r] = t_term;
        }
        CED_DIAG_TICK(6);
        const int64_t start = workgroup_reserve<kWaves>(n, [&](int run) {
            return (long long)atomicAdd(reinterpret_cast<unsigned long long *>(&plan->total_samples), (unsigned long long)run);
        });
        if (active) {
            A.packed[2 * r] = (int32_t)start;
            A.packed[2 * r + 1] = n;
            float *const p0 = A.t_starts + start, *const p1 = A.t_ends + start;
            int32_t *const pr = A.ray_idx + start;
            const auto store = [&](int i, float t0, float t1) { p0[i] = t0; p1[i] = t1; pr[i] = (int32_t)r; };
            if (n > 0 && !runs.replayable(grid)) {
                float unused;
                (void)walk(store, unused);
            } else {
                runs.replay(grid, store);
            }
        }
        CED_DIAG_TICK(7);
        __syncthreads();
    }
#ifdef CED_MARCH_DIAG
    ced_diag_flush();
#endif
}

#ifdef CED_MARCH_DIAG
}
extern "C" int ced_diag_march_read(unsigned long long *out, int reset)
{
    if (hipDeviceSynchronize() != hipSuccess) return -1;
    if (out && hipMemcpyFromSymbol(out, HIP_SYMBOL(g_march_diag), sizeof(unsigned long long) * 24) != hipSuccess) return -1;
    if (reset) {
        unsigned long long z[24] = { 0 };
        if (hipMemcpyToSymbol(HIP_SYMBOL(g_march_diag), z, sizeof(z)) != hipSuccess) return -1;
    }
    return 0;
}
extern "C" int ced_diag_march_waves(unsigned int *out, int max_rows, int reset)
{
    if (hipDeviceSynchronize() != hipSuccess) return -1;
    unsigned int n = 0;
    if (hipMemcpyFromSymbol(&n, HIP_SYMBOL(g_march_wave_n), 4) != hipSuccess) return -1;
    if (n > (unsigned)kDiagWaves) n = kDiagWaves;
    if ((int)n > max_rows) n = max_rows;
    if (out && n && hipMemcpyFromSymbol(out, HIP_SYMBOL(g_march_wave_log), (size_t)n * 96) != hipSuccess) return -1;
    if (reset) {
        unsigned int z = 0;
        if (hipMemcpyToSymbol(HIP_SYMBOL(g_march_wave_n), &z, 4) != hipSuccess) return -1;
    }
    return (int)n;
}
namespace ced {
#endif

__global__ __launch_bounds__(kCompositeThreads) void frame_composite_kernel(
    IterPlan *plan, int n_frames, int rays_per_frame, const int32_t *__restrict__ alive_list,
    int32_t *__restrict__ next_list, const int32_t *__restrict__ packed, const float *__restrict__ t0,
    const float *__restrict__ t1, const float *__restrict__ sig, const float *__restrict__ rgbs, float *__restrict__ rgb,
    float *__restrict__ opacity, float *__restrict__ depth, float opc_thres)
{
    const IterPlan &P = *plan;
    const int64_t total = P.total_slots;
    for (int64_t s0 = (int64_t)blockIdx.x * kCompositeThreads; s0 < total; s0 += (int64_t)gridDim.x * kCompositeThreads) {
        const int f = frame_of_slot(P, n_frames, s0);
        if (f < 0) continue;
        const int limit = P.limit[f];
        const int64_t idx = s0 + threadIdx.x - P.slot_base[f];
        const bool active = idx < P.count[f];
        const int64_t first = (int64_t)f * rays_per_frame;
        const int64_t r = active ? (alive_list ? (int64_t)alive_list[first + idx] : first + idx) : 0;
        int cnt = 0;
        bool alive = false;
        if (active) {
            const int64_t sb = packed[2 * r];
            cnt = packed[2 * r + 1];
            float op = opacity[r];
            if (cnt > 0) {
                const float prefix = 1.0f - op;
                float c0 = rgb[3 * r], c1 = rgb[3 * r + 1], c2 = rgb[3 * r + 2], dp = depth[r];
                float acc = 0.0f;
                constexpr int kU = 4;
                int64_t i = sb;
                const int64_t end = sb + cnt;
                for (; i + kU <= end; i += kU) {
                    float ts[kU], te[kU], sg[kU], cr[kU], cg[kU], cb[kU];
#pragma unroll
                    for (int u = 0; u < kU; ++u) {
                        ts[u] = t0[i + u]; te[u] = t1[i + u]; sg[u] = sig[i + u];
                        cr[u] = rgbs[3 * (i + u)]; cg[u] = rgbs[3 * (i + u) + 1]; cb[u] = rgbs[3 * (i + u) + 2];
                    }
#pragma unroll
                    for (int u = 0; u < kU; ++u) {
                        float sd = sg[u] * (te[u] - ts[u]);
                        float a = 1.0f - det_expf(-sd);
                        float t = det_expf(-acc) * prefix;
                        float w = t * a;
                        c0 = c0 + w * cr[u];
                        c1 = c1 + w * cg[u];
                        c2 = c2 + w * cb[u];
                        op = op + w;
                        dp = dp + w * ((ts[u] + te[u]) / 2.0f);
                        acc = acc + sd;
                    }
                }
                for (; i < end; ++i) {
                    float ts = t0[i], te = t1[i];
                    float sd = sig[i] * (te - ts);
                    float a = 1.0f - det_expf(-sd);
                    float t = det_expf(-acc) * prefix;
                    float w = t * a;
                    c0 = c0 + w * rgbs[3 * i];
                    c1 = c1 + w * rgbs[3 * i + 1];
                    c2 = c2 + w * rgbs[3 * i + 2];
                    op = op + w;
                    dp = dp + w * ((ts + te) / 2.0f);
                    acc = acc + sd;
                }
                rgb[3 * r] = c0; rgb[3 * r + 1] = c1; rgb[3 * r + 2] = c2;
                opacity[r] = op;
                depth[r] = dp;
            }
            alive = !P.last[f] && (op <= opc_thres) && (cnt == limit);
        }
        const int slot = workgroup_append<kCompositeThreads / 64, 1>(alive, &cnt, [&](int run, const int *samples) {
            const unsigned long long add = (unsigned long long)run + ((unsigned long long)samples[0] << 32);
            return add != 0 ? (int)(atomicAdd(&plan->next[f], add) & 0xffffffffull) : 0;
        });
        if (alive) next_list[first + slot] = (int32_t)r;
        __syncthreads();
    }
}

__global__ __launch_bounds__(64) void frame_schedule_kernel(ScheduleArgs S)
{
    make_next_plan(S);
}

__global__ __launch_bounds__(64) void frame_pack_counts_kernel(const IterPlan *__restrict__ plan, int n_frames,
                                                               int64_t *__restrict__ row)
{
    const int f = threadIdx.x;
    if (f >= n_frames) return;
    const unsigned long long nx = __hip_atomic_load(&plan->next[f], __ATOMIC_RELAXED, __HIP_MEMORY_SCOPE_AGENT);
    const bool finished = plan->last[f] || plan->gcount[f] == 0 || plan->count[f] == 0;
    row[f] = finished ? 0 : (int64_t)(nx & 0xffffffffull);
}

__global__ __launch_bounds__(256) void frame_finalize_kernel(int64_t n_rays, const float *__restrict__ bkgd,
                                                             float *__restrict__ rgb, const float *__restrict__ opacity,
                                                             float *__restrict__ depth)
{
    int64_t r = (int64_t)blockIdx.x * blockDim.x + threadIdx.x;
    if (r >= n_rays) return;
    float op = opacity[r];
    if (bkgd) {
        float rem = 1.0f - op;
        rgb[3 * r] = rgb[3 * r] + bkgd[0] * rem;
        rgb[3 * r + 1] = rgb[3 * r + 1] + bkgd[1] * rem;
        rgb[3 * r + 2] = rgb[3 * r + 2] + bkgd[2] * rem;
    }
    depth[r] = depth[r] / __builtin_fmaxf(op, FLT_EPSILON);
}

struct ImageState {
    int32_t *cursor;
    float *acc_all;
    float *acc_kept;
    int32_t *kept;
};

__global__ __launch_bounds__(256) void image_prep_kernel(int64_t n_rays, ImageState st, float *__restrict__ rgb,
                                                         float *__restrict__ opacity, float *__restrict__ depth)
{
    int64_t r = (int64_t)blockIdx.x * blockDim.x + threadIdx.x;
    if (r >= n_rays) return;
    st.cursor[r] = 0; st.acc_all[r] = 0.0f; st.acc_kept[r] = 0.0f; st.kept[r] = 0;
    if (rgb) {
        rgb[3 * r] = 0.0f; rgb[3 * r + 1] = 0.0f; rgb[3 * r + 2] = 0.0f;
        opacity[r] = 0.0f;
        depth[r] = 0.0f;
    }
}

__device__ __forceinline__ int64_t ray_count(const int64_t *__restrict__ packed_all, int64_t r, int64_t n_all)
{
    const int64_t start = packed_all[2 * r], cnt = packed_all[2 * r + 1];
    return (start < 0 || cnt < 0 || start + cnt > n_all) ? 0 : cnt;
}

__global__ __launch_bounds__(kMarchThreads) void image_chunk_kernel(
    IterPlan *__restrict__ plan, int64_t n_all, const int32_t *__restrict__ alive, const int64_t *__restrict__ packed_all,
    const float *__restrict__ t0_all, const float *__restrict__ t1_all, const int32_t *__restrict__ cursor,
    float *__restrict__ t0s, float *__restrict__ t1s, int32_t *__restrict__ ridx, int32_t *__restrict__ packed)
{
    const IterPlan &P = *plan;
    const int64_t total = P.count[0];
    const int limit = P.limit[0];
    const int64_t base = P.sample_base;
    for (int64_t s0 = (int64_t)blockIdx.x * kMarchThreads; s0 < total; s0 += (int64_t)gridDim.x * kMarchThreads) {
        const int64_t idx = s0 + threadIdx.x;
        const bool active = idx < total;
        const int64_t r = active ? (alive ? (int64_t)alive[idx] : idx) : 0;
        int n = 0;
        int64_t src = 0;
        if (active) {
            const int cur = cursor[r];
            const int64_t left = ray_count(packed_all, r, n_all) - cur;
            n = (int)(left < limit ? left : limit);
            src = packed_all[2 * r] + cur;
        }
        const int64_t slot = workgroup_reserve<kMarchThreads / 64>(n, [&](int run) {
            return (long long)atomicAdd(reinterpret_cast<unsigned long long *>(&plan->total_samples), (unsigned long long)run);
        });
        if (active) {
            const int64_t start = base + slot;
            packed[2 * r] = (int32_t)start;
            packed[2 * r + 1] = n;
            for (int i = 0; i < n; ++i) {
                t0s[start + i] = t0_all[src + i];
                t1s[start + i] = t1_all[src + i];
                ridx[start + i] = (int32_t)r;
            }
        }
        __syncthreads();
    }
}

template <bool FULL>
__global__ __launch_bounds__(kCompositeThreads) void image_composite_kernel(
    IterPlan *plan, const int32_t *__restrict__ alive_list, int32_t *__restrict__ next_list,
    const int32_t *__restrict__ packed, const int64_t *__restrict__ packed_all, const float *__restrict__ t0,
    const float *__restrict__ t1, const float *__restrict__ sig, const float *__restrict__ rgbs, ImageState st,
    float *__restrict__ w_out, float *__restrict__ tr_out, float *__restrict__ al_out, int32_t *__restrict__ rank_out,
    float *__restrict__ rgb, float *__restrict__ opacity, float *__restrict__ depth, float eps, float alpha_thre,
    int64_t n_all)
{
    const IterPlan &P = *plan;
    const int64_t total = P.count[0];
    for (int64_t s0 = (int64_t)blockIdx.x * kCompositeThreads; s0 < total; s0 += (int64_t)gridDim.x * kCompositeThreads) {
        const int64_t idx = s0 + threadIdx.x;
        const bool active = idx < total;
        const int64_t r = active ? (alive_list ? (int64_t)alive_list[idx] : idx) : 0;
        int cnt = 0, kept_new = 0;
        bool alive = false;
        if (active) {
            const int64_t sb = packed[2 * r];
            cnt = packed[2 * r + 1];
            if (cnt > 0) {
                float c0 = 0.0f, c1 = 0.0f, c2 = 0.0f, op = 0.0f, dp = 0.0f;
                if constexpr (FULL) { c0 = rgb[3 * r]; c1 = rgb[3 * r + 1]; c2 = rgb[3 * r + 2]; op = opacity[r]; dp = depth[r]; }
                float acc = st.acc_all[r], acck = st.acc_kept[r];
                int kept = st.kept[r];
                const int kept_before = kept;
                bool open = true;
                constexpr int kU = 4;
                const int64_t end = sb + cnt;
                for (int64_t i = sb; i < end; i += kU) {
                    float ts[kU], te[kU], sg[kU], cr[kU], cg[kU], cb[kU];
#pragma unroll
                    for (int u = 0; u < kU; ++u) {
                        const int64_t j = i + u < end ? i + u : end - 1;
                        ts[u] = t0[j]; te[u] = t1[j]; sg[u] = sig[j];
                        if constexpr (FULL) { cr[u] = rgbs[3 * j]; cg[u] = rgbs[3 * j + 1]; cb[u] = rgbs[3 * j + 2]; }
                    }
#pragma unroll
                    for (int u = 0; u < kU; ++u) {
// ... 29 lines not shown
                }
                const int cur = st.cursor[r] + cnt;
                st.cursor[r] = cur;
                st.acc_all[r] = acc; st.acc_kept[r] = acck; st.kept[r] = kept;
                kept_new = kept - kept_before;
                alive = open && (int64_t)cur < ray_count(packed_all, r, n_all) && (det_expf(-acc) >= eps);
            }
        }
        const int sums[2] = { cnt, kept_new };
        const int slot = workgroup_append<kCompositeThreads / 64, 2>(alive, sums, [&](int run, const int *tot) {
            const unsigned long long add = (unsigned long long)run + ((unsigned long long)tot[0] << 32);
            const int base = add != 0 ? (int)(atomicAdd(&plan->next[0], add) & 0xffffffffull) : 0;
            if (tot[1]) atomicAdd(&plan->next[1], (unsigned long long)tot[1]);
            return base;
        });
        if (alive) next_list[slot] = (int32_t)r;
        __syncthreads();
    }
}

struct ImageOut {
    int64_t *ray_indices;
    float *t_starts, *t_ends, *sigmas, *rgbs, *weights, *trans, *alphas;
};

__global__ __launch_bounds__(256) void image_gather_kernel(int64_t n, const int32_t *__restrict__ rank,
                                                           const int32_t *__restrict__ ridx, const float *__restrict__ t0,
                                                           const float *__restrict__ t1, const float *__restrict__ sig,
                                                           const float *__restrict__ rgbs, const float *__restrict__ w,
                                                           const float *__restrict__ tr, const float *__restrict__ al,
                                                           const int64_t *__restrict__ ray_offset, int64_t chunk_rays,
                                                           ImageOut out)
{
    for (int64_t i = (int64_t)blockIdx.x * blockDim.x + threadIdx.x; i < n; i += (int64_t)gridDim.x * blockDim.x) {
        const int k = rank[i];
        if (k < 0) continue;
        const int64_t r = ridx[i];
        const int64_t d = ray_offset[r] + k;
        out.ray_indices[d] = chunk_rays > 0 ? r % chunk_rays : r;
        out.t_starts[d] = t0[i]; out.t_ends[d] = t1[i];
        if (out.sigmas) out.sigmas[d] = sig[i];
        if (out.rgbs) {
            out.rgbs[3 * d] = rgbs[3 * i]; out.rgbs[3 * d + 1] = rgbs[3 * i + 1]; out.rgbs[3 * d + 2] = rgbs[3 * i + 2];
            out.weights[d] = w[i]; out.trans[d] = tr[i]; out.alphas[d] = al[i];
        }
    }
}

struct MarchAllArgs {
    int64_t n_rays;
    const float *rays_o, *rays_d;
    GridSpec grid;
    AccelSpec accel;
    const float *near_planes;
    float far_plane;
    const float *t_sorted;
    const int64_t *t_indices;
    const uint8_t *hits;
    int64_t *packed;
    float *t_starts, *t_ends;
    int64_t *ray_indices;
};

template <bool SINGLE, bool FILL>
__global__ __launch_bounds__(kMarchThreads, SINGLE ? 4 : 3) void march_all_kernel(MarchAllArgs A)
{
    const int64_t r = (int64_t)blockIdx.x * kMarchThreads + threadIdx.x;
    if (r >= A.n_rays) return;
    float o[3], d[3];
#pragma unroll
    for (int a = 0; a < 3; ++a) { o[a] = A.rays_o[3 * r + a]; d[a] = A.rays_d[3 * r + a]; }
    const int m = A.grid.n_grids;
    const float *const ts_row = SINGLE ? nullptr : A.t_sorted + r * 2 * m;
    const int64_t *const ti_row = SINGLE ? nullptr : A.t_indices + r * 2 * m;
    const uint8_t *const hit_row = SINGLE ? nullptr : A.hits + r * m;
    float t_term;
    if constexpr (!FILL) {
        const int n = traverse_ray_frame<kFrameLook, SINGLE, false>(A.grid, A.accel, true, o, d, A.near_planes[r], A.far_plane, ts_row,
                                                             ti_row, hit_row, [](int, float, float) {}, t_term);
        A.packed[2 * r + 1] = n;
    } else {
        const int64_t start = A.packed[2 * r];
        if (A.packed[2 * r + 1] == 0) return;
        float *const p0 = A.t_starts + start, *const p1 = A.t_ends + start;
        int64_t *const pr = A.ray_indices ? A.ray_indices + start : nullptr;
        (void)traverse_ray_frame<kFrameLook, SINGLE, false>(A.grid, A.accel, true, o, d, A.near_planes[r], A.far_plane, ts_row, ti_row,
                                                     hit_row,
                                                     [&](int i, float t0, float t1) {
                                                         p0[i] = t0; p1[i] = t1;
                                                         if (pr) pr[i] = r;
                                                     },
                                                     t_term);
    }
}

template <bool SINGLE>
__global__ __launch_bounds__(kMarchThreads, SINGLE ? 4 : 3) void march_all_onepass_kernel(MarchAllArgs A, int64_t capacity,
                                                                                         unsigned long long *total)
{
    const int64_t r = (int64_t)blockIdx.x * kMarchThreads + threadIdx.x;
    const bool active = r < A.n_rays;
    const int m = A.grid.n_grids;
    float o[3] = { 0.0f, 0.0f, 0.0f }, d[3] = { 0.0f, 0.0f, 1.0f };
    float near = 0.0f, t_term = 0.0f;
    const float *const ts_row = (SINGLE || !active) ? nullptr : A.t_sorted + r * 2 * m;
    const int64_t *const ti_row = (SINGLE || !active) ? nullptr : A.t_indices + r * 2 * m;
    const uint8_t *const hit_row = (SINGLE || !active) ? nullptr : A.hits + r * m;
    const auto walk = [&](auto &&emit, float &t_out) {
        return traverse_ray_frame<kFrameLook, SINGLE, false>(A.grid, A.accel, true, o, d, near, A.far_plane, ts_row, ti_row,
                                                             hit_row, emit, t_out);
    };
    SampleRuns runs;
    int n = 0;
    if (active) {
#pragma unroll
        for (int a = 0; a < 3; ++a) { o[a] = A.rays_o[3 * r + a]; d[a] = A.rays_d[3 * r + a]; }
        near = A.near_planes[r];
        n = walk([&](int i, float t0, float t1) { runs.record(i, t0, t1); }, t_term);
    }
    const int64_t start = workgroup_reserve<kMarchThreads / 64>(n, [&](int run) {
        return (long long)atomicAdd(total, (unsigned long long)run);
    });
    if (!active) return;
    A.packed[2 * r] = start;
    A.packed[2 * r + 1] = n;
    if (n == 0 || start + n > capacity) return;
    float *const p0 = A.t_starts + start, *const p1 = A.t_ends + start;
    const auto store = [&](int i, float t0, float t1) { p0[i] = t0; p1[i] = t1; };
    if (!runs.replayable(A.grid)) {
        float unused;
        (void)walk(store, unused);
    } else {
        runs.replay(A.grid, store);
    }
}

struct Carver {
    char *base;
    size_t off = 0;
    template <class T> T *take(size_t count)
    {
        T *p = (T *)(base + off);
        off = (off + count * sizeof(T) + 255) & ~(size_t)255;
        return p;
    }
};

struct FrameWorkspace {
    float *t_sorted; uint8_t *t_indices; uint8_t *hits; float *near; int32_t *packed;
    int32_t *alive_a, *alive_b;
    IterPlan *plans;
    float *lattice;
    float *ts_ray;
    float *t0, *t1; int32_t *ridx; float *sigma, *rgbs;
    uint8_t *accel;
    size_t bytes;
};

static inline int min_samples_of(float cone_angle) { return cone_angle == 0.0f ? 1 : 4; }
static inline int max_iterations(int max_samples, int min_samples) { return (max_samples + min_samples - 1) / min_samples; }

static inline int64_t sample_capacity(int n_frames, int64_t rays_per_frame, int min_samples, int64_t global_rays)
{
    int64_t per = rays_per_frame * min_samples;
    if (global_rays > rays_per_frame) {
        const int64_t worst = rays_per_frame * 64 < global_rays ? rays_per_frame * 64 : global_rays;
        if (worst > per) per = worst;
    }
    return per * n_frames;
}

static FrameWorkspace carve(void *base, int64_t n, int m, int64_t cap, int max_iters, int res, bool per_ray_times = false)
{
    FrameWorkspace w{};
    Carver c{ (char *)base };
    w.t_sorted = c.take<float>((size_t)n * 2 * m);
    w.t_indices = c.take<uint8_t>((size_t)n * 2 * m);
    w.hits = c.take<uint8_t>((size_t)n * m);
    w.near = c.take<float>((size_t)n);
    w.packed = c.take<int32_t>((size_t)n * 2);
    w.alive_a = c.take<int32_t>((size_t)n);
    w.alive_b = c.take<int32_t>((size_t)n);
    w.plans = c.take<IterPlan>((size_t)max_iters + 2);
    w.lattice = c.take<float>(256);
    w.ts_ray = c.take<float>(per_ray_times ? (size_t)n : 0);
    w.t0 = c.take<float>((size_t)cap);
    w.t1 = c.take<float>((size_t)cap);
    w.ridx = c.take<int32_t>((size_t)cap);
    w.sigma = c.take<float>((size_t)cap);
    w.rgbs = c.take<float>((size_t)cap * 3);
    const int64_t nbk = (res + kBrick - 1) / kBrick;
    w.accel = c.take<uint8_t>((size_t)(2 * m * nbk * nbk * nbk));
    w.bytes = c.off;
    return w;
}

static std::atomic<long long> g_publish_seq{ 0 };

#if defined(__HIP_DEVICE_COMPILE__)
#define CED_CPU_PAUSE()
#else
#define CED_CPU_PAUSE() __builtin_ia32_pause()
#endif

static int wait_published(volatile long long *flag, long long seq, hipStream_t stream, const char *who)
{
    const auto t_start = std::chrono::steady_clock::now();
    long spins = 0;
    while (__atomic_load_n(flag, __ATOMIC_ACQUIRE) < seq) {
        if ((++spins & 0x3ff) == 0) {
            if (std::chrono::steady_clock::now() - t_start > std::chrono::milliseconds(200)) {
                if (hipStreamSynchronize(stream) != hipSuccess) return check_launch("render_image_test (sync)");
                if (__atomic_load_n(flag, __ATOMIC_ACQUIRE) < seq) {
                    set_error("%s: iteration %lld was not published although the stream has drained", who, seq);
                    return CED_E_LAUNCH;
                }
                break;
            }
        } else {
            CED_CPU_PAUSE();
        }
    }
    return CED_OK;
}

static int run_ahead(volatile long long *pub, volatile long long *host_iter, const std::vector<long long> &plan_seq, int it,
                     hipStream_t stream, const char *who, bool &stop, long long &alive_bound)
{
    const int need = it - kRunAhead;
    if (need < 0 && host_iter) return CED_OK;
    volatile long long *const rec = host_iter ? host_iter + 3 * need : pub;
    if (need >= 0) {
        const int rc = wait_published(rec + 2, plan_seq[need], stream, who);
        if (rc) return rc;
    }
    if (host_iter || __atomic_load_n(pub + 2, __ATOMIC_ACQUIRE) >= plan_seq[0]) {
        if (rec[1]) {
            stop = true;
            return CED_OK;
        }
        const long long a = rec[0];
        if (a >= 0 && a < alive_bound) alive_bound = a;
    }
    return CED_OK;
}

static int read_back_plans(const IterPlan *dev_plans, int enqueued, hipStream_t stream, const char *what, const char *who,
                           std::vector<IterPlan> &plans, int &n_iters)
{
    plans.resize((size_t)enqueued + 1);
    if (hipMemcpyAsync(plans.data(), dev_plans, plans.size() * sizeof(IterPlan), hipMemcpyDeviceToHost, stream) != hipSuccess ||
        hipStreamSynchronize(stream) != hipSuccess)
        return check_launch(what);
    n_iters = 0;
    while (n_iters < enqueued && !plans[n_iters].done && plans[n_iters].total_slots != 0) ++n_iters;
    if (n_iters == enqueued && !plans[enqueued].done) {
        set_error("%s: the loop stopped after %d iterations with rays still alive", who, enqueued);
        return CED_E_LAUNCH;
    }
    return CED_OK;
}

static int render_frames_impl(const ced_field_desc *field, int n_frames, int64_t rays_per_frame, const float *rays_o,
                              const float *rays_d, const uint8_t *binaries, int32_t n_grids, int32_t res,
                              const float *aabbs, const void *accel, float near_plane, float far_plane, float step_size,
                              float cone_angle, float early_stop_eps, int32_t max_samples, const float *timestamps,
                              int32_t t_per_ray, const float *frame_times, const float *bkgd, float *rgb, float *opacity,
                              float *depth, void *workspace, int64_t workspace_bytes, int64_t *host_stats,
                              int64_t *total_samples_out, ced_frame_trace *trace, void *field_stream_, void *stream_,
                              const char *who, const ced_shard_exchange *xch = nullptr)
{
    hipStream_t stream = (hipStream_t)stream_;
    hipStream_t fstream = field_stream_ ? (hipStream_t)field_stream_ : stream;
    const bool split = fstream != stream;
    constexpr int kMaxDevices = 64;
    static thread_local hipEvent_t ev_to_field[kMaxDevices] = {}, ev_from_field[kMaxDevices] = {};
    int dev = 0;
    if (split) {
        if (hipGetDevice(&dev) != hipSuccess || dev < 0 || dev >= kMaxDevices) return check_launch("render_image_test (device)");
        if (!ev_to_field[dev] &&
            (hipEventCreateWithFlags(&ev_to_field[dev], hipEventDisableTiming) != hipSuccess ||
             hipEventCreateWithFlags(&ev_from_field[dev], hipEventDisableTiming) != hipSuccess))
            return check_launch("render_image_test (event create)");
    }
    const int64_t n_rays = (int64_t)n_frames * rays_per_frame;
    CED_REQUIRE(field != nullptr, "%s: null field descriptor", who);
    CED_REQUIRE(n_frames >= 1 && n_frames <= kMaxFrames, "%s: n_frames must be 1..%d", who, kMaxFrames);
    CED_REQUIRE(rays_per_frame >= 0 && n_grids >= 1 && n_grids <= kMaxGrids && res >= 1 && res <= 1024, "%s: bad sizes", who);
    CED_REQUIRE(n_rays < (1ll << 31) / 4, "%s: too many rays for 32-bit sample indices", who);
    CED_REQUIRE(max_samples >= 0, "%s: max_samples < 0", who);
    if (total_samples_out)
        for (int f = 0; f < n_frames; ++f) total_samples_out[f] = 0;
    if (trace) trace->n_iters = 0;
    if (n_rays == 0) return CED_OK;
    CED_REQUIRE(rays_o && rays_d && binaries && aabbs && (timestamps || frame_times) && rgb && opacity && depth &&
                    workspace && host_stats,
                "%s: null pointer", who);
    const int min_samples = min_samples_of(cone_angle);
    const int64_t cap = sample_capacity(n_frames, rays_per_frame, min_samples, xch ? xch->global_rays_per_frame : 0);
    CED_REQUIRE(cap < (1ll << 31) - 64, "%s: too many samples per iteration for 32-bit sample indices", who);
    const int max_iters = max_iterations(max_samples, min_samples);
    FrameWorkspace W = carve(workspace, n_rays, n_grids, cap, max_iters, res, frame_times != nullptr);
    CED_REQUIRE((int64_t)W.bytes <= workspace_bytes, "%s: workspace too small (%lld < %lld bytes)", who,
                (long long)workspace_bytes, (long long)W.bytes);
    if (xch) {
        CED_REQUIRE(xch->reduce && xch->counts && xch->global_rays_per_frame >= rays_per_frame &&
                        xch->global_rays_per_frame < (1ll << 31),
                    "%s: bad ced_shard_exchange (reduce / counts NULL, or global_rays_per_frame < rays_per_frame)", who);
        CED_REQUIRE(!field_stream_ || field_stream_ == stream_, "%s: a sharded call takes no separate field stream", who);
    }
    long long *const host_iter = xch ? (long long *)host_stats + kHostIterWord : nullptr;
    const dim3 blk(256), grd((unsigned)((n_rays + 255) / 256));

    if (n_grids == 1)
        hipLaunchKernelGGL(frame_prep_single_kernel, grd, blk, 0, stream, n_rays, near_plane, W.near, rgb, opacity, depth);
    else
        hipLaunchKernelGGL(frame_prep_kernel, grd, blk, 0, stream, n_rays, rays_o, rays_d, (int)n_grids, aabbs, near_plane,
                           W.t_sorted, W.t_indices, W.hits, W.near, rgb, opacity, depth);
    if (frame_times)
        hipLaunchKernelGGL(frame_times_kernel, grd, blk, 0, stream, n_rays, (int)rays_per_frame, frame_times, W.ts_ray);
    const int nb = (res + kBrick - 1) / kBrick;
    AccelSpec acc;
    if (accel) {
        acc = accel_view(accel, n_grids, res, true);
    } else {
        int rc = build_brick_accel(binaries, n_grids, res, W.accel, W.accel + (size_t)n_grids * nb * nb * nb, stream);
        if (rc) return rc;
        acc = AccelSpec{ W.accel, nb, nullptr };
    }
    volatile long long *pub = (volatile long long *)host_stats;
    std::vector<long long> plan_seq((size_t)max_iters + 1);
    plan_seq[0] = ++g_publish_seq;
    const bool use_lattice = cone_angle == 0.0f && step_size > 0.0f && near_plane >= 0.0f;
    if (use_lattice) build_lattice(near_plane, step_size, reinterpret_cast<float *>(host_stats + kHostLatticeWord));
    hipLaunchKernelGGL(frame_init_kernel, dim3(1), dim3(64), 0, stream,
                       ScheduleArgs{ W.plans, -1, n_frames, (int)rays_per_frame, min_samples, (int)max_samples,
                                     (long long *)host_stats, plan_seq[0], xch ? xch->local_rays : nullptr, nullptr,
                                     xch ? xch->global_rays_per_frame : 0, host_iter },
                       use_lattice ? W.lattice : (float *)nullptr,
                       (unsigned long long *)(trace ? trace->field_stamps : nullptr),
                       (trace && trace->field_stamps) ? (int)trace->capacity : 0);
    int rc = check_launch("render_image_test (prep)");
    if (rc) return rc;

    const float opc_thres = (float)(1.0 - (double)early_stop_eps);
    long long alive_bound = n_rays;
    int it = 0;
    for (; it < max_iters; ++it) {
        bool stop = false;
        rc = run_ahead(pub, host_iter, plan_seq, it, stream, who, stop, alive_bound);
        if (rc) return rc;
        if (stop) break;
        IterPlan *plan = W.plans + it;
        const int32_t *cur_list = it == 0 ? nullptr : ((it & 1) ? W.alive_a : W.alive_b);
        int32_t *next_list = (it & 1) ? W.alive_b : W.alive_a;

        const int64_t slot_bound = alive_bound + (int64_t)n_frames * kSlotAlign;
        MarchArgs M{ rays_o, rays_d, GridSpec{ binaries, aabbs, n_grids, res, step_size, cone_angle, 0, use_lattice ? W.lattice : nullptr },
                     acc, W.near, far_plane, cur_list, n_frames,
                     (int)rays_per_frame, W.t_sorted, W.t_indices, W.hits, W.t0, W.t1, W.ridx, W.packed, W.alive_b };
        int64_t mgrid = (slot_bound + kMarchThreads - 1) / kMarchThreads;
        if (mgrid > 8192) mgrid = 8192;
        const dim3 mblk(kMarchThreads);
        const int two_pass_opt = g_march_two_pass;
        const bool two_pass = two_pass_opt < 0 ? n_grids > 1 : two_pass_opt != 0;
        if (it == 0 && acc.bdist && two_pass) {
            int64_t kgrid = (slot_bound + kCullThreads - 1) / kCullThreads;
            if (kgrid > 8192) kgrid = 8192;
            if (mgrid > 4096) mgrid = 4096;
            if (n_grids == 1) {
                hipLaunchKernelGGL(march_cull_kernel<true>, dim3((unsigned)kgrid), dim3(kCullThreads), 0, stream, M, plan);
                hipLaunchKernelGGL((march_frame_kernel<true, true, true>), dim3((unsigned)mgrid), mblk, 0, stream, M, plan);
            } else {
                hipLaunchKernelGGL(march_cull_kernel<false>, dim3((unsigned)kgrid), dim3(kCullThreads), 0, stream, M, plan);
                hipLaunchKernelGGL((march_frame_kernel<false, true, true>), dim3((unsigned)mgrid), mblk, 0, stream, M, plan);
            }
        } else if (it == 0) {
            if (n_grids == 1) hipLaunchKernelGGL((march_frame_kernel<true, false, true>), dim3((unsigned)mgrid), mblk, 0, stream, M, plan);
            else hipLaunchKernelGGL((march_frame_kernel<false, false, true>), dim3((unsigned)mgrid), mblk, 0, stream, M, plan);
        } else {
            if (n_grids == 1) hipLaunchKernelGGL((march_frame_kernel<true, false, false>), dim3((unsigned)mgrid), mblk, 0, stream, M, plan);
            else hipLaunchKernelGGL((march_frame_kernel<false, false, false>), dim3((unsigned)mgrid), mblk, 0, stream, M, plan);
        }
        rc = check_launch("render_image_test (march)");
        if (rc) return rc;

        FieldArgs F{};
        F.n = cap;
        F.n_dev = &plan->total_samples;
        F.rays_o = rays_o; F.rays_d = rays_d; F.ray_idx32 = W.ridx;
        F.t0 = W.t0; F.t1 = W.t1;
        F.timestamps = frame_times ? W.ts_ray : timestamps;
        F.rays_mode = 1; F.t_per_ray = (frame_times || t_per_ray) ? 1 : 0; F.want_rgb = 1;
        F.rgb = W.rgbs; F.sigma = W.sigma; F.geo = nullptr;
        if (trace && trace->field_stamps && it < trace->capacity)
            F.stamp = reinterpret_cast<unsigned long long *>(trace->field_stamps) + 2 * it;
        if (split) {
            (void)hipEventRecord(ev_to_field[dev], stream);
            (void)hipStreamWaitEvent(fstream, ev_to_field[dev], 0);
        }
        if (trace && it < trace->capacity && trace->field_begin)
            (void)hipEventRecord((hipEvent_t)trace->field_begin[it], fstream);
        rc = launch_field(field, F, (void *)fstream);
        if (rc) return rc;
        if (trace && it < trace->capacity && trace->field_end)
            (void)hipEventRecord((hipEvent_t)trace->field_end[it], fstream);
        if (split) {
            (void)hipEventRecord(ev_from_field[dev], fstream);
            (void)hipStreamWaitEvent(stream, ev_from_field[dev], 0);
        }

        int64_t cgrid = (slot_bound + kCompositeThreads - 1) / kCompositeThreads;
        if (cgrid > 4096) cgrid = 4096;
        plan_seq[it + 1] = ++g_publish_seq;
        hipLaunchKernelGGL(frame_composite_kernel, dim3((unsigned)cgrid), dim3(kCompositeThreads), 0, stream,
                           plan, n_frames, (int)rays_per_frame, cur_list, next_list, W.packed, W.t0, W.t1, W.sigma, W.rgbs,
                           rgb, opacity, depth, opc_thres);
        int64_t *xrow = nullptr;
        if (xch) {
            xrow = xch->counts + (int64_t)it * n_frames;
            hipLaunchKernelGGL(frame_pack_counts_kernel, dim3(1), dim3(64), 0, stream, plan, n_frames, xrow);
            rc = check_launch("render_image_test (pack counts)");
            if (rc) return rc;
            const int xrc = xch->reduce(xch->user, xrow, n_frames, it, (void *)stream);
            if (xrc != 0) {
                set_error("%s: the exchange step of iteration %d failed (code %d)", who, it, xrc);
                (void)hipStreamSynchronize(stream);
                return CED_E_LAUNCH;
            }
        }
        hipLaunchKernelGGL(frame_schedule_kernel, dim3(1), dim3(64), 0, stream,
                           ScheduleArgs{ W.plans, it, n_frames, (int)rays_per_frame, min_samples, (int)max_samples,
                                         (long long *)host_stats, plan_seq[it + 1], xch ? xch->local_rays : nullptr,
                                         xch ? xch->counts : nullptr, xch ? xch->global_rays_per_frame : 0, host_iter });
        rc = check_launch("render_image_test (composite / schedule)");
        if (rc) return rc;
    }
    const int enqueued = it;
    hipLaunchKernelGGL(frame_finalize_kernel, grd, blk, 0, stream, n_rays, bkgd, rgb, opacity, depth);
    rc = check_launch("render_image_test (finalize)");
    if (rc) return rc;
    std::vector<IterPlan> plans;
    int n_iters = 0;
    rc = read_back_plans(W.plans, enqueued, stream, "render_image_test (read-back)", who, plans, n_iters);
    if (rc) return rc;
    int64_t total[kMaxFrames] = { 0 };
    for (int k = 0; k < n_iters; ++k) {
        const IterPlan &P = plans[k];
        int64_t alive_total = 0, samples_it = 0;
        int max_limit = 0;
        for (int f = 0; f < n_frames; ++f) {
            alive_total += P.count[f];
            samples_it += (int64_t)(P.next[f] >> 32);
            total[f] += (int64_t)(P.next[f] >> 32);
            if (P.count[f] > 0 && P.limit[f] > max_limit) max_limit = P.limit[f];
        }
        if (trace && k < trace->capacity) {
            if (trace->iter_alive) trace->iter_alive[k] = alive_total;
            if (trace->iter_n_samples) trace->iter_n_samples[k] = max_limit;
            if (trace->iter_samples) trace->iter_samples[k] = samples_it;
        }
    }
    if (trace) trace->n_iters = n_iters;
    if (total_samples_out)
        for (int f = 0; f < n_frames; ++f) total_samples_out[f] = total[f];
    return CED_OK;
}

struct ImageWorkspace {
    ImageState st;
    int32_t *packed, *alive_a, *alive_b;
    IterPlan *plans;
    float *t0, *t1; int32_t *ridx; float *sigma, *rgbs, *w, *tr, *al; int32_t *rank;
    size_t bytes;
};

constexpr int kImageMaxIters = 1024;

static ImageWorkspace carve_image(void *base, int64_t n, int64_t cap)
{
    ImageWorkspace w{};
    Carver c{ (char *)base };
    w.st.cursor = c.take<int32_t>((size_t)n);
    w.st.acc_all = c.take<float>((size_t)n);
    w.st.acc_kept = c.take<float>((size_t)n);
    w.packed = c.take<int32_t>((size_t)n * 2);
    w.alive_a = c.take<int32_t>((size_t)n);
    w.alive_b = c.take<int32_t>((size_t)n);
    w.plans = c.take<IterPlan>((size_t)kImageMaxIters + 2);
    w.t0 = c.take<float>((size_t)cap);
    w.t1 = c.take<float>((size_t)cap);
    w.ridx = c.take<int32_t>((size_t)cap);
    w.sigma = c.take<float>((size_t)cap);
    w.rgbs = c.take<float>((size_t)cap * 3);
    w.w = c.take<float>((size_t)cap);
    w.tr = c.take<float>((size_t)cap);
    w.al = c.take<float>((size_t)cap);
    w.rank = c.take<int32_t>((size_t)cap);
    w.bytes = c.off;
    return w;
}

static inline int64_t image_capacity(int64_t n_rays, int64_t n_all) { return n_all + 64; }

static int render_image_impl(const ced_field_desc *field, int64_t n_rays, const float *rays_o, const float *rays_d,
                             int64_t n_all, const int64_t *packed_all, const float *t0_all, const float *t1_all,
                             float early_stop_eps, float alpha_thre, const float *timestamps, int32_t t_per_ray,
                             const float *bkgd, float *rgb, float *opacity, float *depth, int32_t *kept, void *workspace,
                             int64_t workspace_bytes, int64_t *host_stats, int64_t *stats_out, void *field_stream_,
                             void *stream_)
{
    const char *who = "render_image";
    hipStream_t stream = (hipStream_t)stream_;
    hipStream_t fstream = field_stream_ ? (hipStream_t)field_stream_ : stream;
    CED_REQUIRE(fstream == stream, "%s: a separate field stream is not supported", who);
    CED_REQUIRE(field != nullptr, "%s: null field descriptor", who);
    CED_REQUIRE(n_rays >= 0 && n_all >= 0, "%s: bad sizes", who);
    CED_REQUIRE(n_rays < (1ll << 31) / 4 && n_all < (1ll << 31) - 128, "%s: too many rays / samples for 32-bit indices", who);
    if (stats_out) { stats_out[0] = 0; stats_out[1] = 0; stats_out[2] = 0; }
    if (n_rays == 0) return CED_OK;
    const bool full = rgb != nullptr;
    CED_REQUIRE(rays_o && rays_d && packed_all && (n_all == 0 || (t0_all && t1_all)) && timestamps && kept && workspace &&
                    host_stats && (!full || (opacity && depth)),
                "%s: null pointer", who);
    const int64_t cap = image_capacity(n_rays, n_all);
    ImageWorkspace W = carve_image(workspace, n_rays, cap);
    W.st.kept = kept;
    CED_REQUIRE((int64_t)W.bytes <= workspace_bytes, "%s: workspace too small (%lld < %lld bytes)", who,
                (long long)workspace_bytes, (long long)W.bytes);
    const dim3 blk(256), grd((unsigned)((n_rays + 255) / 256));
    hipLaunchKernelGGL(image_prep_kernel, grd, blk, 0, stream, n_rays, W.st, rgb, opacity, depth);
    volatile long long *pub = (volatile long long *)host_stats;
    std::vector<long long> plan_seq((size_t)kImageMaxIters + 1);
    plan_seq[0] = ++g_publish_seq;
    const int big = 1 << 30;
    const int min_chunk = full ? 4 : 8;
    hipLaunchKernelGGL(frame_init_kernel, dim3(1), dim3(64), 0, stream,
                       ScheduleArgs{ W.plans, -1, 1, (int)n_rays, min_chunk, big, (long long *)host_stats, plan_seq[0] }, (float *)nullptr,
                       (unsigned long long *)nullptr, 0);
    int rc = check_launch("render_image (prep)");
    if (rc) return rc;
    long long alive_bound = n_rays;
    int it = 0;
    for (; it < kImageMaxIters; ++it) {
        bool stop = false;
        rc = run_ahead(pub, nullptr, plan_seq, it, stream, who, stop, alive_bound);
        if (rc) return rc;
        if (stop) break;
        IterPlan *plan = W.plans + it;
        const int32_t *cur_list = it == 0 ? nullptr : ((it & 1) ? W.alive_a : W.alive_b);
        int32_t *next_list = (it & 1) ? W.alive_b : W.alive_a;
        int64_t mgrid = (alive_bound + kMarchThreads - 1) / kMarchThreads;
        if (mgrid > 8192) mgrid = 8192;
        if (mgrid < 1) mgrid = 1;
        hipLaunchKernelGGL(image_chunk_kernel, dim3((unsigned)mgrid), dim3(kMarchThreads), 0, stream, plan, n_all, cur_list,
                           packed_all, t0_all, t1_all, W.st.cursor, W.t0, W.t1, W.ridx, W.packed);
        FieldArgs F{};
        F.n = n_rays * (int64_t)min_chunk;
        F.n_dev = &plan->total_samples;
        F.base_dev = &plan->sample_base;
        F.rays_o = rays_o; F.rays_d = rays_d; F.ray_idx32 = W.ridx;
        F.t0 = W.t0; F.t1 = W.t1;
        F.timestamps = timestamps;
        F.rays_mode = 1; F.t_per_ray = t_per_ray ? 1 : 0; F.want_rgb = full ? 1 : 0;
        F.rgb = full ? W.rgbs : nullptr; F.sigma = W.sigma; F.geo = nullptr;
        rc = launch_field(field, F, (void *)stream);
        if (rc) return rc;
        int64_t cgrid = (alive_bound + kCompositeThreads - 1) / kCompositeThreads;
        if (cgrid > 4096) cgrid = 4096;
// ... 208 lines not shown
```

ced_nerf_amd/ops.py:

```python
from __future__ import annotations

import ctypes as C
from typing import Dict, Optional, Tuple

import numpy as np
import torch

from . import _lib, profiling
from .hashgrid import level_tables


def _stream() -> C.c_void_p:
    return C.c_void_p(torch.cuda.current_stream().cuda_stream)


def _chk(t: Optional[torch.Tensor], dtype: torch.dtype, name: str, allow_none: bool = False):
    if t is None:
        if allow_none:
            return None
        raise ValueError(f"{name} is required")
    if not t.is_cuda:
        raise NotImplementedError(f"Only support cuda inputs ({name} is on {t.device}).")
    _check_current_device(t.device.index, name)
    if t.dtype != dtype:
# ... 56 lines not shown
        raise ValueError(f"weight shapes {got} do not match the DNGPradianceField layout {want}")
    if mlp_precision == _lib.MLP_F32_HEAD16X2:
        n = int(L.ced_packed_weight_floats(int(use_div_offsets), int(time_mode)))
        out = np.zeros((n,), np.float32)
        rc = L.ced_pack_field_weights_mixed(int(use_div_offsets), int(time_mode),
                                            *[m.ctypes.data_as(C.c_void_p) for m in mats], out.ctypes.data_as(C.c_void_p))
        _lib.check(rc, "pack_field_weights_mixed")
        return out
    if mlp_precision != _lib.MLP_F32:
        n = int(L.ced_packed_weight_words(int(use_div_offsets), int(time_mode), int(mlp_precision)))
        if n <= 0:
            raise ValueError(f"mlp_precision={mlp_precision}")
        out = np.zeros((n,), np.uint32)
        rc = L.ced_pack_field_weights_half_for(int(use_div_offsets), int(time_mode), int(mlp_precision), int(table_dtype),
                                               int(bool(temporal)), *[m.ctypes.data_as(C.c_void_p) for m in mats],
                                               out.ctypes.data_as(C.c_void_p))
        _lib.check(rc, "pack_field_weights_half_for")
        return out
    n = int(L.ced_packed_weight_floats(int(use_div_offsets), int(time_mode)))
    out = np.zeros((n,), np.float32)
    rc = L.ced_pack_field_weights(int(use_div_offsets), int(time_mode),
                                  *[m.ctypes.data_as(C.c_void_p) for m in mats], out.ctypes.data_as(C.c_void_p))
    _lib.check(rc, "pack_field_weights")
    return out


def ray_aabb_intersect(rays_o, rays_d, aabbs, near_plane=-float("inf"), far_plane=float("inf"),
                       miss_value=float("inf")):
    _chk(rays_o, torch.float32, "rays_o"); _chk(rays_d, torch.float32, "rays_d"); _chk(aabbs, torch.float32, "aabbs")
    assert rays_o.ndim == 2 and rays_o.shape[-1] == 3 and rays_o.shape == rays_d.shape
    assert aabbs.ndim == 2 and aabbs.shape[-1] == 6
    n, m = rays_o.shape[0], aabbs.shape[0]
    t_mins = torch.empty((n, m), device=rays_o.device, dtype=torch.float32)
    t_maxs = torch.empty_like(t_mins)
    hits = torch.empty((n, m), device=rays_o.device, dtype=torch.bool)
    rc = _lib.lib().ced_ray_aabb_intersect(n, _p(rays_o), _p(rays_d), m, _p(aabbs), near_plane, far_plane,
                                           miss_value, _p(t_mins), _p(t_maxs), _p(hits), _stream())
    _lib.check(rc, "ray_aabb_intersect")
    return t_mins, t_maxs, hits


def sort_intersections(t_mins, t_maxs):
    _chk(t_mins, torch.float32, "t_mins"); _chk(t_maxs, torch.float32, "t_maxs")
    assert t_mins.ndim == 2 and t_mins.shape == t_maxs.shape
    n, m = t_mins.shape
    t_sorted = torch.empty((n, 2 * m), device=t_mins.device, dtype=torch.float32)
    t_indices = torch.empty((n, 2 * m), device=t_mins.device, dtype=torch.int64)
    rc = _lib.lib().ced_sort_intersections(n, m, _p(t_mins), _p(t_maxs), _p(t_sorted), _p(t_indices), _stream())
    _lib.check(rc, "sort_intersections")
    return t_sorted, t_indices


def traverse_grids_raw(rays_o, rays_d, binaries, aabbs, near_planes, far_planes, step_size, cone_angle, limit,
                       rays_mask, t_sorted, t_indices, hits, mode, base=None, counts=None, t_starts=None,
                       t_ends=None, ray_indices=None, termination_planes=None, packed_info_out=None):
    L = _lib.lib()
    n = rays_o.shape[0]
    m, res = binaries.shape[0], binaries.shape[1]
    with profiling.span("traverse", n):
        rc = L.ced_traverse_grids(n, _p(rays_o), _p(rays_d), _p(_as_u8(binaries)), m, res, _p(aabbs), _p(near_planes),
                                  _p(far_planes), float(step_size), float(cone_angle), int(limit),
                                  _p(_as_u8(rays_mask)), _p(t_sorted), _p(t_indices), _p(_as_u8(hits)), int(mode),
                                  _p(base), _p(counts), _p(t_starts), _p(t_ends), _p(ray_indices),
                                  _p(termination_planes), _p(packed_info_out), _stream())
    _lib.check(rc, "traverse_grids")


def hash_encode(desc: _lib.HashDesc, x: torch.Tensor, t: Optional[torch.Tensor] = None) -> torch.Tensor:
    _chk(x, torch.float32, "x")
    assert x.ndim == 2 and x.shape[-1] == 3
    if t is not None:
        _chk(t, torch.float32, "t")
        assert t.numel() == x.shape[0]
    out = torch.empty((x.shape[0], 2 * desc.n_levels), device=x.device, dtype=torch.float32)
    rc = _lib.lib().ced_hash_encode(C.byref(desc), x.shape[0], _p(x), _p(t), _p(out), _stream())
    _lib.check(rc, "hash_encode")
    return out


def hash_encode_backward(desc: _lib.HashDesc, x: torch.Tensor, dy: torch.Tensor,
                         grad_table: Optional[torch.Tensor] = None, want_dx: bool = True, dx_scaled: bool = False,
                         want_table: bool = True):
    _chk(x, torch.float32, "x"); _chk(dy, torch.float32, "dy")
    n = x.shape[0]
    assert x.shape == (n, 3) and dy.numel() == n * 2 * desc.n_levels, f"{x.shape} v.s. {dy.shape}"
    assert want_table or want_dx
    if not want_table:
        grad_table = None
    elif grad_table is None:
        grad_table = torch.zeros((int(desc.total_entries), 2), device=x.device, dtype=torch.float32)
    else:
        _chk(grad_table, torch.float32, "grad_table")
        assert grad_table.shape == (int(desc.total_entries), 2)
    dx = torch.empty((n, 3), device=x.device, dtype=torch.float32) if want_dx else None
    rc = _lib.lib().ced_hash_encode_backward(C.byref(desc), n, _p(x), _p(dy), _p(grad_table), _p(dx), int(dx_scaled),
                                             _stream())
    _lib.check(rc, "hash_encode_backward")
    return grad_table, dx


def hash_encode_backward_temporal(desc: _lib.HashDesc, x: torch.Tensor, t: torch.Tensor, dy: torch.Tensor,
                                  grad_table: Optional[torch.Tensor] = None) -> torch.Tensor:
    _chk(x, torch.float32, "x"); _chk(dy, torch.float32, "dy"); _chk(t, torch.float32, "t")
    n = x.shape[0]
    assert desc.temporal, "not a temporal table"
    assert x.shape == (n, 3) and t.numel() == n and dy.numel() == n * 2 * desc.n_levels, f"{x.shape} {t.shape} {dy.shape}"
    if grad_table is None:
        grad_table = torch.zeros((int(desc.total_entries), 8), device=x.device, dtype=torch.float32)
    else:
        _chk(grad_table, torch.float32, "grad_table")
        assert grad_table.shape == (int(desc.total_entries), 8)
    rc = _lib.lib().ced_hash_encode_backward_temporal(C.byref(desc), n, _p(x), _p(t), _p(dy), _p(grad_table), _stream())
    _lib.check(rc, "hash_encode_backward_temporal")
    return grad_table


def field_forward(desc: _lib.FieldDesc, positions, t, directions=None, want_geo=False):
    _chk(positions, torch.float32, "positions"); _chk(t, torch.float32, "t")
    n = positions.shape[0]
    assert positions.shape == (n, 3) and t.numel() == n
    dev = positions.device
    rgb = None
    if directions is not None:
        _chk(directions, torch.float32, "directions")
        assert directions.shape == positions.shape, f"{positions.shape} v.s. {directions.shape}"
        rgb = torch.empty((n, 3), device=dev, dtype=torch.float32)
    sigma = torch.empty((n,), device=dev, dtype=torch.float32)
    geo = torch.empty((n, 15), device=dev, dtype=torch.float32) if want_geo else None
    rc = _lib.lib().ced_field_forward(C.byref(desc), n, _p(positions), _p(t), _p(directions), _p(rgb), _p(sigma),
                                      _p(geo), _stream())
    _lib.check(rc, "field_forward")
    return rgb, sigma, geo


def field_forward_rays(desc: _lib.FieldDesc, rays_o, rays_d, ray_indices, t_starts, t_ends, timestamps,
                       t_per_ray: bool, want_rgb: bool, n_dev: Optional[torch.Tensor] = None):
    _chk(rays_o, torch.float32, "rays_o"); _chk(rays_d, torch.float32, "rays_d")
    _chk(ray_indices, torch.int64, "ray_indices")
    _chk(t_starts, torch.float32, "t_starts"); _chk(t_ends, torch.float32, "t_ends")
    _chk(timestamps, torch.float32, "timestamps")
    n = ray_indices.shape[0]
    assert t_starts.shape == (n,) and t_ends.shape == (n,)
    if t_per_ray:
        assert timestamps.numel() == rays_o.shape[0], "per-ray timestamps must have one entry per ray"
    dev = rays_o.device
    rgb = torch.empty((n, 3), device=dev, dtype=torch.float32) if want_rgb else None
    sigma = torch.empty((n,), device=dev, dtype=torch.float32)
    with profiling.span("field", n):
        rc = _lib.lib().ced_field_forward_rays(C.byref(desc), n, _p(n_dev), _p(rays_o), _p(rays_d), _p(ray_indices),
                                               _p(t_starts), _p(t_ends), _p(timestamps), int(bool(t_per_ray)),
                                               int(bool(want_rgb)), _p(rgb), _p(sigma), _stream())
    _lib.check(rc, "field_forward_rays")
    return rgb, sigma


def field_move(desc: _lib.FieldDesc, positions, t, want=(True, True, True, True)):
    _chk(positions, torch.float32, "positions"); _chk(t, torch.float32, "t")
    n = positions.shape[0]
    assert positions.shape == (n, 3) and t.numel() == n
    if not any(want):
        raise ValueError("field_move: no output requested")
    dev = positions.device
    outs = [torch.empty((n, 3), device=dev, dtype=torch.float32) if w else None for w in want[:3]]
    sel = torch.empty((n,), device=dev, dtype=torch.bool) if want[3] else None
    rc = _lib.lib().ced_field_move(C.byref(desc), n, _p(positions), _p(t), _p(outs[0]), _p(outs[1]), _p(outs[2]),
                                   _p(_as_u8(sel)), _stream())
    _lib.check(rc, "field_move")
    return outs[0], outs[1], outs[2], sel


def field_move_rays(desc: _lib.FieldDesc, rays_o, rays_d, ray_indices, t_starts, t_ends, timestamps, t_per_ray: bool,
                    want_x_norm: bool = False, n_dev: Optional[torch.Tensor] = None, out=None):
    _chk(rays_o, torch.float32, "rays_o"); _chk(rays_d, torch.float32, "rays_d")
    _chk(ray_indices, torch.int64, "ray_indices")
    _chk(t_starts, torch.float32, "t_starts"); _chk(t_ends, torch.float32, "t_ends")
    _chk(timestamps, torch.float32, "timestamps")
    n = ray_indices.shape[0]
    assert t_starts.shape == (n,) and t_ends.shape == (n,)
    if t_per_ray:
        assert timestamps.numel() == rays_o.shape[0], "per-ray timestamps must have one entry per ray"
    dev = rays_o.device
    if out is not None:
        move, x_norm = out
        _chk(move, torch.float32, "out[0]"); _chk(x_norm, torch.float32, "out[1]", allow_none=True)
        assert move.shape == (n, 3) and (x_norm is None or x_norm.shape == (n, 3))
    else:
        move = torch.empty((n, 3), device=dev, dtype=torch.float32)
        x_norm = torch.empty((n, 3), device=dev, dtype=torch.float32) if want_x_norm else None
    rc = _lib.lib().ced_field_move_rays(C.byref(desc), n, _p(n_dev), _p(rays_o), _p(rays_d), _p(ray_indices), _p(t_starts),
                                        _p(t_ends), _p(timestamps), int(bool(t_per_ray)), _p(move), _p(x_norm), _stream())
    _lib.check(rc, "field_move_rays")
    return move, x_norm


MAX_SOLVE_ITERS = 1024


def check_solve(max_iters, tol):
    if isinstance(max_iters, bool) or not isinstance(max_iters, (int, np.integer)) or not 1 <= int(max_iters) <= MAX_SOLVE_ITERS:
        raise ValueError(f"max_iters must be an int in 1 .. {MAX_SOLVE_ITERS}, got {max_iters!r}")
    try:
        tol_f = float(tol)
    except (TypeError, ValueError):
        raise ValueError(f"tol must be a number >= 0, got {tol!r}") from None
    if not tol_f >= 0.0:
        raise ValueError(f"tol must be a number >= 0, got {tol!r}")
    return int(max_iters), tol_f


SOLVE_METHODS = ("fixed_point", "newton")


def check_method(method) -> str:
    if method not in SOLVE_METHODS:
        raise ValueError(f"method must be one of {SOLVE_METHODS}, got {method!r}")
    return method


def _move_inverse(entry: str, desc, target, t, init, max_iters, tol):
    max_iters, tol = check_solve(max_iters, tol)
    _chk(target, torch.float32, "target"); _chk(t, torch.float32, "t"); _chk(init, torch.float32, "init", allow_none=True)
    n = target.shape[0]
    if target.shape != (n, 3) or t.numel() != n or (init is not None and init.shape != (n, 3)):
        raise ValueError(f"target [n,3], t [n], init [n,3]: got {list(target.shape)}, {list(t.shape)}, "
                         f"{None if init is None else list(init.shape)}")
    dev = target.device
    x = torch.empty((n, 3), device=dev, dtype=torch.float32)
    step = torch.empty((n,), device=dev, dtype=torch.float32)
    evals = torch.empty((n,), device=dev, dtype=torch.int32)
    rc = getattr(_lib.lib(), "ced_" + entry)(C.byref(desc), n, _p(target), _p(t), _p(init), max_iters, tol, _p(x), _p(step),
                                             _p(evals), _stream())
    _lib.check(rc, entry)
    return x, step, evals


def _track(entry: str, desc, target, times, init, max_iters, tol):
    max_iters, tol = check_solve(max_iters, tol)
    _chk(target, torch.float32, "target"); _chk(times, torch.float32, "times")
    _chk(init, torch.float32, "init", allow_none=True)
    p, nt = target.shape[0], times.shape[0]
    if target.shape != (p, 3) or times.shape != (nt,) or (init is not None and init.shape != (p, 3)):
        raise ValueError(f"target [P,3], times [T], init [P,3]: got {list(target.shape)}, {list(times.shape)}, "
                         f"{None if init is None else list(init.shape)}")
    dev = target.device
    x = torch.empty((nt, p, 3), device=dev, dtype=torch.float32)
    step = torch.empty((nt, p), device=dev, dtype=torch.float32)
    evals = torch.empty((nt, p), device=dev, dtype=torch.int32)
    rc = getattr(_lib.lib(), "ced_" + entry)(C.byref(desc), p, nt, _p(target), _p(times), _p(init), max_iters, tol, _p(x),
                                             _p(step), _p(evals), _stream())
    _lib.check(rc, entry)
    return x, step, evals


def field_move_inverse(desc: _lib.FieldDesc, target, t, init=None, max_iters: int = 32, tol: float = 1e-6):
    return _move_inverse("field_move_inverse", desc, target, t, init, max_iters, tol)


def field_track(desc: _lib.FieldDesc, target, times, init=None, max_iters: int = 32, tol: float = 1e-6):
    return _track("field_track", desc, target, times, init, max_iters, tol)


def field_move_jacobian(desc: _lib.FieldDesc, positions, t, want=(True, True)):
    _chk(positions, torch.float32, "positions"); _chk(t, torch.float32, "t")
    n = positions.shape[0]
    if positions.shape != (n, 3) or t.numel() != n:
        raise ValueError(f"positions [n,3], t [n]: got {list(positions.shape)}, {list(t.shape)}")
    if not any(want):
        raise ValueError("field_move_jacobian: no output requested")
    dev = positions.device
    move = torch.empty((n, 3), device=dev, dtype=torch.float32) if want[0] else None
    jac = torch.empty((n, 3, 4), device=dev, dtype=torch.float32) if want[1] else None
    rc = _lib.lib().ced_field_move_jacobian(C.byref(desc), n, _p(positions), _p(t), _p(move), _p(jac), _stream())
    _lib.check(rc, "field_move_jacobian")
    return move, jac


def field_move_inverse_newton(desc: _lib.FieldDesc, target, t, init=None, max_iters: int = 32, tol: float = 1e-6):
    return _move_inverse("field_move_inverse_newton", desc, target, t, init, max_iters, tol)


def field_track_newton(desc: _lib.FieldDesc, target, times, init=None, max_iters: int = 32, tol: float = 1e-6):
    return _track("field_track_newton", desc, target, times, init, max_iters, tol)


def warp_gradient(jac: torch.Tensor):
    A = jac[..., :3] + torch.eye(3, device=jac.device, dtype=jac.dtype)
    rows = [torch.linalg.cross(A[..., (a + 1) % 3, :], A[..., (a + 2) % 3, :], dim=-1) for a in range(3)]
    cof = torch.stack(rows, -2)
    det = (A[..., 0, :] * cof[..., 0, :]).sum(-1)
    return A, cof.transpose(-1, -2) / det[..., None, None], det


def field_rgb(desc: _lib.FieldDesc, directions, embedding, apply_act: bool = True):
    _chk(directions, torch.float32, "directions"); _chk(embedding, torch.float32, "embedding")
    n = directions.shape[0]
    assert directions.shape == (n, 3) and embedding.shape == (n, 15), f"{directions.shape} v.s. {embedding.shape}"
    rgb = torch.empty((n, 3), device=directions.device, dtype=torch.float32)
    rc = _lib.lib().ced_field_rgb(C.byref(desc), n, _p(directions), _p(embedding), int(bool(apply_act)), _p(rgb), _stream())
    _lib.check(rc, "field_rgb")
    return rgb


def field_rgb_bcast(desc: _lib.FieldDesc, directions, embedding, apply_act: bool = True):
    _chk(directions, torch.float32, "directions"); _chk(embedding, torch.float32, "embedding")
    m, d = embedding.shape[0], directions.shape[0]
    assert directions.shape == (d, 3) and embedding.shape == (m, 15), f"{directions.shape} v.s. {embedding.shape}"
# ... 830 lines not shown
```

include/cednerf_hip.h:

```cpp
#ifndef CEDNERF_HIP_H
#define CEDNERF_HIP_H

#include <stddef.h>
#include <stdint.h>

#ifdef __cplusplus
extern "C" {
#endif

#define CED_MAX_LEVELS 16

#define CED_OK 0
#define CED_E_INVALID (-1)
#define CED_E_LAUNCH (-2)
#define CED_E_UNSUPPORTED (-3)

typedef struct ced_hash_desc {
    int32_t n_levels;
    int32_t table_dtype;
    int32_t temporal;
    int32_t reserved;
    float scale[CED_MAX_LEVELS];
    uint32_t res[CED_MAX_LEVELS];
    uint32_t offset[CED_MAX_LEVELS];
    uint32_t size[CED_MAX_LEVELS];
    uint32_t hashed[CED_MAX_LEVELS];
    const void *table;
    uint64_t total_entries;
} ced_hash_desc;

typedef struct ced_field_desc {
    float aabb[6];
    float moving_step;
    int32_t use_div_offsets;
    int32_t time_mode;
    int32_t mlp_precision;
    int32_t max_workgroups;
    const void *packed_weights;
    uint64_t packed_floats;
    ced_hash_desc hash;
} ced_field_desc;

int ced_version(void);
const char *ced_last_error_string(void);

int ced_set_option(const char *key, int value);

#define CED_MLP_F32 0
#define CED_MLP_F16X2 1
#define CED_MLP_F16 2
#define CED_MLP_F32_HEAD16X2 3

int64_t ced_packed_weight_floats(int use_div_offsets, int time_mode);

int ced_pack_field_weights(int use_div_offsets, int time_mode,
                           const float *m_w0, const float *m_w1, const float *m_w2, const float *m_w3,
                           const float *b_w0, const float *b_w1,
                           const float *h_w0, const float *h_w1, const float *h_w2,
                           float *out);

int64_t ced_packed_weight_words(int use_div_offsets, int time_mode, int mlp_precision);
int ced_pack_field_weights_half(int use_div_offsets, int time_mode, int mlp_precision,
                                const float *m_w0, const float *m_w1, const float *m_w2, const float *m_w3,
                                const float *b_w0, const float *b_w1,
                                const float *h_w0, const float *h_w1, const float *h_w2,
                                void *out);
int ced_pack_field_weights_half_for(int use_div_offsets, int time_mode, int mlp_precision, int table_dtype, int temporal,
                                    const float *m_w0, const float *m_w1, const float *m_w2, const float *m_w3,
                                    const float *b_w0, const float *b_w1,
                                    const float *h_w0, const float *h_w1, const float *h_w2,
                                    void *out);
int ced_pack_field_weights_mixed(int use_div_offsets, int time_mode,
                                 const float *m_w0, const float *m_w1, const float *m_w2, const float *m_w3,
                                 const float *b_w0, const float *b_w1,
                                 const float *h_w0, const float *h_w1, const float *h_w2,
                                 float *out);

int ced_ray_aabb_intersect(int64_t n_rays, const float *rays_o, const float *rays_d,
                           int32_t n_aabbs, const float *aabbs,
                           float near_plane, float far_plane, float miss_value,
                           float *t_mins, float *t_maxs, uint8_t *hits, void *stream);

int ced_sort_intersections(int64_t n_rays, int32_t n_grids, const float *t_mins, const float *t_maxs, float *t_sorted,
                           int64_t *t_indices, void *stream);

int ced_traverse_grids(int64_t n_rays, const float *rays_o, const float *rays_d,
                       const uint8_t *binaries, int32_t n_grids, int32_t res, const float *aabbs,
                       const float *near_planes, const float *far_planes,
                       float step_size, float cone_angle, int32_t limit, const uint8_t *rays_mask,
                       const float *t_sorted, const int64_t *t_indices, const uint8_t *hits,
                       int32_t mode, const int64_t *base,
                       int64_t *counts, float *t_starts, float *t_ends, int64_t *ray_indices,
                       float *termination_planes, int64_t *packed_info_out, void *stream);

int64_t ced_occupancy_accel_bytes(int32_t n_grids, int32_t res);
int ced_build_occupancy_accel(const uint8_t *binaries, int32_t n_grids, int32_t res, void *accel, int64_t accel_bytes,
                              void *stream);

int ced_host_build_occupancy_accel(const uint8_t *binaries_host, int32_t n_grids, int32_t res, uint8_t *accel_host);
int32_t ced_host_count_steps(float *x, float d, float tau, int32_t kcap, float *prev);
int ced_host_march_frame(int64_t n_rays, const float *rays_o, const float *rays_d, const uint8_t *binaries,
                         int32_t n_grids, int32_t res, const float *aabbs, const float *near_planes, float far_plane,
                         float step_size, float cone_angle, int32_t limit, const float *t_sorted,
                         const int64_t *t_indices, const uint8_t *hits, const uint8_t *accel_host, int32_t accel_mode,
                         int32_t use_lattice, int32_t start_coarse, int32_t *counts, float *t_starts, float *t_ends,
                         float *t_term);

float ced_host_skip_march(float t_last, float target, float step_size, float cone_angle);

int ced_hash_encode(const ced_hash_desc *desc, int64_t n, const float *x, const float *t,
                    float *out, void *stream);

int ced_hash_encode_backward(const ced_hash_desc *desc, int64_t n, const float *x, const float *dy,
                             float *grad_table, float *dx, int32_t dx_scaled, void *stream);

int ced_hash_encode_backward_temporal(const ced_hash_desc *desc, int64_t n, const float *x, const float *t,
                                      const float *dy, float *grad_table, void *stream);

int ced_field_forward(const ced_field_desc *desc, int64_t n, const float *positions, const float *t,
                      const float *directions, float *rgb, float *sigma, float *geo, void *stream);

int ced_field_forward_rays(const ced_field_desc *desc, int64_t n, const int64_t *n_dev,
                           const float *rays_o, const float *rays_d,
                           const int64_t *ray_indices, const float *t_starts, const float *t_ends,
                           const float *timestamps, int32_t t_per_ray, int32_t want_rgb,
                           float *rgb, float *sigma, void *stream);

int ced_field_move(const ced_field_desc *desc, int64_t n, const float *positions, const float *t,
                   float *x_move, float *move, float *x_norm, uint8_t *selector, void *stream);

int ced_field_move_rays(const ced_field_desc *desc, int64_t n, const int64_t *n_dev,
                        const float *rays_o, const float *rays_d,
                        const int64_t *ray_indices, const float *t_starts, const float *t_ends,
                        const float *timestamps, int32_t t_per_ray, float *move, float *x_norm, void *stream);

int ced_field_move_inverse(const ced_field_desc *desc, int64_t n, const float *target, const float *t,
                           const float *init, int32_t max_iters, float tol, float *x, float *step,
                           int32_t *evals, void *stream);

int ced_field_track(const ced_field_desc *desc, int64_t n_points, int64_t n_times, const float *target,
                    const float *times, const float *init, int32_t max_iters, float tol, float *x,
                    float *step, int32_t *evals, void *stream);

int ced_field_move_jacobian(const ced_field_desc *desc, int64_t n, const float *positions, const float *t,
                            float *move, float *jac, void *stream);

int ced_field_move_inverse_newton(const ced_field_desc *desc, int64_t n, const float *target, const float *t,
                                  const float *init, int32_t max_iters, float tol, float *x, float *step,
                                  int32_t *evals, void *stream);

int ced_field_track_newton(const ced_field_desc *desc, int64_t n_points, int64_t n_times, const float *target,
                           const float *times, const float *init, int32_t max_iters, float tol, float *x,
                           float *step, int32_t *evals, void *stream);

int ced_field_rgb(const ced_field_desc *desc, int64_t n, const float *dirs, const float *embedding,
                  int32_t apply_act, float *rgb, void *stream);

int ced_field_rgb_bcast(const ced_field_desc *desc, int64_t m, int32_t n_dirs, const float *dirs,
                        const float *embedding, int32_t apply_act, float *rgb, void *stream);

int64_t ced_bake_workspace_bytes(int64_t n);

int ced_bake_candidates(int32_t reso, const float *center_host, float radius, int64_t first_cell, int64_t n_cells,
                        const uint8_t *binaries, const float *aabbs, int32_t levels, int32_t grid_res,
                        int64_t capacity, int64_t *index, float *xyz, int64_t *count, void *workspace,
                        int64_t workspace_bytes, void *stream);

int ced_bake_select(int64_t n, const int64_t *index_in, const float *xyz_in, const float *sigma_in,
                    const float *embedding_in, float sigma_thresh, int64_t capacity, int64_t *index, float *xyz,
                    float *sigma, float *embedding, int64_t *count, void *workspace, int64_t workspace_bytes,
                    void *stream);

int64_t ced_mesh_workspace_bytes(int32_t reso);

int ced_mesh_vertices(int32_t reso, const float *center_host, float radius, const float *lattice, float thresh,
                      int64_t capacity, float *vertices, float *normals, int64_t *cube, int64_t *count,
                      void *workspace, int64_t workspace_bytes, void *stream);

int ced_mesh_faces(int32_t reso, const float *lattice, float thresh, const int64_t *cube, int64_t n_vertices,
                   int64_t capacity, int32_t *faces, int64_t *count, void *workspace, int64_t workspace_bytes,
                   void *stream);

int ced_render_weights(int64_t n_rays, const int64_t *packed_info, const float *t_starts,
                       const float *t_ends, const float *sigmas, const float *prefix_trans,
                       float *weights, float *trans, float *alphas, void *stream);

int ced_accumulate_along_rays(int64_t n_rays, const int64_t *packed_info, const float *weights,
                              const float *values, int32_t n_channels, float *out, void *stream);

int ced_reduce_along_rays(int64_t n_samples, const int64_t *ray_indices, const float *values, int32_t n_channels,
                          const float *weights, int32_t weight_channels, int64_t n_rays, int32_t mean, float *out,
                          int32_t *counts_workspace, void *stream);

int ced_visibility_mask(int64_t n_rays, const int64_t *packed_info, const float *t_starts,
                        const float *t_ends, const float *sigmas, float early_stop_eps, float alpha_thre,
                        uint8_t *mask, void *stream);

int ced_composite_prefix(int64_t n_rays, const int64_t *packed_info, const float *t_starts,
                         const float *t_ends, const float *sigmas, const float *rgbs,
                         float *rgb, float *opacity, float *depth, void *stream);

int ced_composite_backward(int64_t n_rays, const int64_t *packed_info, const float *t_starts,
                           const float *t_ends, const float *sigmas, const float *rgbs,
                           const float *d_color, const float *d_opacity, const float *d_depth,
                           float *d_sigmas, float *d_rgbs, void *stream);

int64_t ced_distortion_workspace_bytes(int64_t n_rays, int64_t n_samples, int32_t density);
int ced_distortion_loss(int64_t n_rays, int64_t n_samples, const int64_t *packed_info, const float *weights,
                        const float *t_starts, const float *t_ends, float *ray_loss, float *grad_weights,
                        void *workspace, float *loss, float *inv_norm, void *stream);
int ced_distortion_loss_density(int64_t n_rays, int64_t n_samples, const int64_t *packed_info, const float *sigmas,
                                const float *t_starts, const float *t_ends, float *ray_loss, float *d_sigmas,
                                void *workspace, float *loss, float *inv_norm, void *stream);

int64_t ced_ssim_workspace_bytes(int64_t n, int64_t c, int64_t h, int64_t w, int32_t win_size, int32_t levels);
int ced_ssim(int64_t n, int64_t c, int64_t h, int64_t w, const float *x, const int64_t *x_strides, const float *y,
             const int64_t *y_strides, double data_range, double k1, double k2, int32_t win_size, const float *win,
             int32_t levels, const float *weights, int32_t nonnegative, float *per_image, float *mean, double *mse,
             double *level_means, void *workspace, void *stream);

int ced_frame_to_rgb8(int32_t height, int32_t width, const float *rgb, int32_t flip_w, uint8_t *out, void *stream);
int ced_depth_to_u8(int32_t height, int32_t width, const float *depth, int32_t flip_w, uint8_t *out,
                    void *workspace, void *stream);

int ced_scatter_pixels(int64_t n_rows, const float *src_rgb, int32_t stride_rgb, const float *src_opacity,
                       int32_t stride_opacity, const float *src_depth, int32_t stride_depth, const int64_t *dest,
                       int64_t n_pixels, float *rgb, float *opacity, float *depth, uint8_t *rgb8, int32_t width,
                       int32_t flip_w, void *stream);

int ced_linear(int64_t n, const float *x, int32_t n_in, const float *w, int32_t w_rows, int32_t w_cols,
               int32_t transpose_w, int32_t n_out, int32_t relu, const float *mask, float *y, void *stream);

int64_t ced_weight_grad_workspace_bytes(int64_t n, int32_t n_out, int32_t n_in);
int ced_weight_grad(int64_t n, const float *x, int32_t n_in, const float *dy, int32_t n_out, float *dw,
                    void *workspace, int64_t workspace_bytes, void *stream);

int ced_composite_step(int64_t n_rays, const int64_t *packed_info, const float *t_starts,
                       const float *t_ends, const float *sigmas, const float *rgbs,
                       float *rgb, float *opacity, float *depth,
                       float opc_thres, int32_t n_samples_iter, uint8_t *ray_mask, int64_t *stats,
                       void *stream);

int ced_composite_test(int64_t n_alive, const float *sigmas, const float *rgbs, const float *t_start,
                       const float *t_end, const int64_t *pack_info, int64_t *alive_indices,
                       float T_threshold, float alpha_threshold,
                       float *opacity, float *depth, float *rgb, void *stream);

int ced_finalize_pixels(int64_t n_rays, const float *bkgd, float *rgb, const float *opacity,
                        float *depth, void *stream);


int ced_occ_cell_points(int64_t n, const int64_t *cell_indices, const float *noise, int32_t res,
                        const float *aabb_host, float *positions, void *stream);

int ced_occ_ema_update(int64_t n, const int64_t *cell_ids, const float *density, float step_size,
                       float ema_decay, float *occs, void *stream);


int ced_generate_rays_pinhole(int32_t width, int32_t height, float fx, float fy, float cx, float cy,
                              const float *c2w_host, int32_t opengl, float *origins, float *viewdirs,
                              float *directions, void *stream);

int ced_generate_rays_hypercam(int32_t width, int32_t height, const float *orientation_host,
                               const float *position_host, float focal_length, float principal_x, float principal_y,
                               float skew, float pixel_aspect_ratio, const float *radial3_host,
                               const float *tangential2_host, float *origins, float *viewdirs, void *stream);

#define CED_CAMERA_PINHOLE 0
#define CED_CAMERA_HYPERCAM 1
#define CED_PINHOLE_FLOATS 17
#define CED_HYPERCAM_FLOATS 22
#define CED_VIEW_PER_RAY 0
#define CED_VIEW_PER_STEP 1
#define CED_BKGD_WHITE 0
#define CED_BKGD_BLACK 1
#define CED_BKGD_RANDOM 2
int ced_sample_training_batch(int32_t camera_model, int32_t n_views, int32_t width, int32_t height, int32_t channels,
                              const uint8_t *images, const float *cameras, const float *view_timestamps,
                              int64_t num_rays, uint64_t seed, int64_t step, int32_t view_mode, int32_t bkgd_mode,
// ... 119 lines not shown
```

Measured before the change: 4.423 billion.

## Pack per-sample march/field/composite buffers into 16-byte AoS records

Replaces the separate t_starts/t_ends/ray_idx arrays with one 16-byte SampleIn record, and the separate sigma/rgb arrays with one 16-byte SampleOut record, across the march, field and composite kernels of the frame renderer. The field kernel reads one vector load per sample and writes all four output channels per lane, including a sigma lane for the fourth group. The composite reads a float2 and a float4 per sample. The aim is fewer, wider, coalesced memory transactions and fewer inter-stage buffers. In exchange the record fields must be 16-byte aligned, and the kernels carry extra branches for the record versus legacy paths.

```diff
diff --git a/ced_nerf_amd/_lib.py b/ced_nerf_amd/_lib.py
--- a/ced_nerf_amd/_lib.py
+++ b/ced_nerf_amd/_lib.py
@@ -84,6 +84,7 @@
     "ced_field_forward": (C.c_int, [C.POINTER(FieldDesc), _i64, _vp, _vp, _vp, _vp, _vp, _vp, _vp]),
     "ced_field_forward_rays": (C.c_int, [C.POINTER(FieldDesc), _i64, _vp, _vp, _vp, _vp, _vp, _vp, _vp, _i32, _i32,
                                          _vp, _vp, _vp]),
+    "ced_field_forward_records": (C.c_int, [C.POINTER(FieldDesc), _i64, _vp, _vp, _vp, _vp, _vp, _i32, _i32, _vp, _vp]),
     "ced_field_move": (C.c_int, [C.POINTER(FieldDesc), _i64, _vp, _vp, _vp, _vp, _vp, _vp, _vp]),
     "ced_field_move_rays": (C.c_int, [C.POINTER(FieldDesc), _i64, _vp, _vp, _vp, _vp, _vp, _vp, _vp, _i32, _vp, _vp, _vp]),
     "ced_field_move_inverse": (C.c_int, [C.POINTER(FieldDesc), _i64, _vp, _vp, _vp, _i32, _f, _vp, _vp, _vp, _vp]),
diff --git a/ced_nerf_amd/csrc/field.hip b/ced_nerf_amd/csrc/field.hip
--- a/ced_nerf_amd/csrc/field.hip
+++ b/ced_nerf_amd/csrc/field.hip
@@ -452,6 +452,27 @@
     return ced::launch_field(desc, A, stream);
 }
 
+extern "C" int ced_field_forward_records(const ced_field_desc *desc, int64_t n, const int64_t *n_dev, const float *rays_o,
+                                         const float *rays_d, const void *records_in, const float *timestamps,
+                                         int32_t t_per_ray, int32_t want_rgb, void *records_out, void *stream)
+{
+    CED_REQUIRE(desc != nullptr, "field_forward_records: null descriptor");
+    CED_REQUIRE(n >= 0, "field_forward_records: n < 0");
+    if (n == 0) return CED_OK;
+    CED_REQUIRE(rays_o && rays_d && records_in && timestamps && records_out, "field_forward_records: null pointer");
+    CED_REQUIRE((((uintptr_t)records_in | (uintptr_t)records_out) & 15) == 0,
+                "field_forward_records: the record arrays must be 16-byte aligned");
+    ced::FieldArgs A{};
+    A.n = n;
+    A.n_dev = n_dev;
+    A.rays_o = rays_o; A.rays_d = rays_d;
+    A.rec_in = static_cast<const ced::SampleIn *>(records_in);
+    A.rec_out = static_cast<ced::SampleOut *>(records_out);
+    A.timestamps = timestamps;
+    A.rays_mode = 1; A.t_per_ray = t_per_ray ? 1 : 0; A.want_rgb = want_rgb ? 1 : 0;
+    return ced::launch_field(desc, A, stream);
+}
+
 extern "C" int ced_hash_encode(const ced_hash_desc *desc, int64_t n, const float *x, const float *t, float *out,
                                void *stream)
 {
diff --git a/ced_nerf_amd/csrc/field_args.hpp b/ced_nerf_amd/csrc/field_args.hpp
--- a/ced_nerf_amd/csrc/field_args.hpp
+++ b/ced_nerf_amd/csrc/field_args.hpp
@@ -6,6 +6,16 @@
 #include "../../include/cednerf_hip.h"
 
 namespace ced {
+
+struct alignas(16) SampleIn {
+    float t0, t1;
+    int32_t ray;
+    int32_t pad;
+};
+struct alignas(16) SampleOut {
+    float r, g, b, sigma;
+};
+static_assert(sizeof(SampleIn) == 16 && sizeof(SampleOut) == 16, "sample records are 16 bytes");
 
 struct FieldArgs {
     int64_t n;
@@ -30,6 +40,8 @@
     const void *table;
     float scale[CED_MAX_LEVELS];
     uint32_t res[CED_MAX_LEVELS], offset[CED_MAX_LEVELS], size[CED_MAX_LEVELS], hashed[CED_MAX_LEVELS];
+    const SampleIn *rec_in;
+    SampleOut *rec_out;
 };
 
 extern std::atomic<int> g_march_two_pass;
diff --git a/ced_nerf_amd/csrc/field_half.hip b/ced_nerf_amd/csrc/field_half.hip
--- a/ced_nerf_amd/csrc/field_half.hip
+++ b/ced_nerf_amd/csrc/field_half.hip
@@ -80,17 +80,29 @@
         int64_t ridx[NT];
         float px[NT][3], tq[NT];
         bool any_used = !A.rays_mode;
-#pragma unroll
-        for (int j = 0; j < NT; ++j) {
+        bool rec_skip[NT];
+#pragma unroll
+        for (int j = 0; j < NT; ++j) {
+            rec_skip[j] = false;
             sofs[j] = 16 * j + c < in_tile ? 16 * j + c : in_tile - 1;
             const int64_t s = tile_base + sofs[j];
             if (A.rays_mode) {
-                const int64_t r_in = A.ray_idx32 ? (int64_t)A.ray_idx32[sbase + s] : A.ray_idx[sbase + s];
+                int64_t r_in;
+                float tsum;
+                if (A.rec_in) {
+                    const SampleIn rec = A.rec_in[sbase + s];
+                    r_in = rec.ray;
+                    tsum = rec.t0 + rec.t1;
+                } else {
+                    r_in = A.ray_idx32 ? (int64_t)A.ray_idx32[sbase + s] : A.ray_idx[sbase + s];
+                    tsum = A.t0[sbase + s] + A.t1[sbase + s];
+                }
                 const bool used = r_in >= 0;
                 const int64_t r = used ? r_in : 0;
                 any_used = any_used || used;
+                rec_skip[j] = A.rec_out && !used;
                 ridx[j] = r;
-                const float tm2 = used ? A.t0[sbase + s] + A.t1[sbase + s] : 0.0f;
+                const float tm2 = used ? tsum : 0.0f;
 #pragma unroll
                 for (int a = 0; a < 3; ++a) px[j][a] = A.rays_o[3 * r + a] + (A.rays_d[3 * r + a] * tm2) / 2.0f;
                 tq[j] = A.t_per_ray ? A.timestamps[r] : A.timestamps[0];
@@ -202,13 +214,19 @@
         to_operand_h<NT, SPLIT>(D, Bh, Bl);
         mlp_layer_h<2, 1, NT, SPLIT, K32>(whi + BL::B1 * kFragHalves, wlo + BL::B1 * kFragHalves, lane, Bh, Bl, D);
 
-#pragma unroll
-        for (int j = 0; j < NT; ++j) {
-            const bool stored = 16 * j + c < in_tile;
+        float sg_rec[NT];
+#pragma unroll
+        for (int j = 0; j < NT; ++j) {
+            const bool stored = 16 * j + c < in_tile && !rec_skip[j];
             const int64_t s = tile_base + (16 * j + c);
             float sg = det_expf(D[j][0][3] - 1.0f);
             sg = sel[j] ? sg : 0.0f;
-            if (g == 3 && stored) A.sigma[sbase + s] = sg;
+            sg_rec[j] = sg;
+            if (A.rec_out) {
+                if (!A.want_rgb && g == 3 && stored) A.rec_out[sbase + s].sigma = sg;
+            } else if (g == 3 && stored) {
+                A.sigma[sbase + s] = sg;
+            }
             if (A.geo && stored) {
 #pragma unroll
                 for (int r = 0; r < 4; ++r)
@@ -246,7 +264,11 @@
             for (int j = 0; j < NT; ++j) {
                 const int64_t s = tile_base + (16 * j + c);
                 const float o1 = 1.0f / (1.0f + det_expf(-D[j][0][0]));
-                if (g < 3 && 16 * j + c < in_tile) A.rgb[3 * (sbase + s) + g] = o1;
+                if (A.rec_out) {
+                    if (16 * j + c < in_tile && !rec_skip[j]) reinterpret_cast<float *>(A.rec_out)[4 * (sbase + s) + g] = g < 3 ? o1 : sg_rec[j];
+                } else if (g < 3 && 16 * j + c < in_tile) {
+                    A.rgb[3 * (sbase + s) + g] = o1;
+                }
             }
         }
     }
diff --git a/ced_nerf_amd/csrc/field_kernel.hpp b/ced_nerf_amd/csrc/field_kernel.hpp
--- a/ced_nerf_amd/csrc/field_kernel.hpp
+++ b/ced_nerf_amd/csrc/field_kernel.hpp
@@ -91,6 +91,13 @@
     }
 }
 
+__device__ __forceinline__ int lane_id_now()
+{
+    unsigned zero = 0;
+    asm volatile("" : "+v"(zero));
+    return (int)__builtin_amdgcn_mbcnt_hi(~0u, __builtin_amdgcn_mbcnt_lo(~0u, zero));
+}
+
 template <bool TE, bool F16, bool TEMPORAL, int NT, int THREADS, bool HEAD16 = false>
 __global__ __launch_bounds__(THREADS) void field_kernel(FieldArgs A)
 {
@@ -144,18 +151,30 @@
         int64_t ridx[NT];
         float px[NT][3], tq[NT];
         bool any_used = !A.rays_mode;
-#pragma unroll
-        for (int j = 0; j < NT; ++j) {
+        bool rec_skip[NT];
+#pragma unroll
+        for (int j = 0; j < NT; ++j) {
+            rec_skip[j] = false;
             int64_t s = tile * TILE + 16 * j + c;
             s = s < n_eff ? s : n_eff - 1;
             sidx[j] = s;
             if (A.rays_mode) {
-                const int64_t r_in = A.ray_idx32 ? (int64_t)A.ray_idx32[sbase + s] : A.ray_idx[sbase + s];
+                int64_t r_in;
+                float tsum;
+                if (A.rec_in) {
+                    const SampleIn rec = A.rec_in[sbase + s];
+                    r_in = rec.ray;
+                    tsum = rec.t0 + rec.t1;
+                } else {
+                    r_in = A.ray_idx32 ? (int64_t)A.ray_idx32[sbase + s] : A.ray_idx[sbase + s];
+                    tsum = A.t0[sbase + s] + A.t1[sbase + s];
+                }
                 const bool used = r_in >= 0;
                 const int64_t r = used ? r_in : 0;
                 any_used = any_used || used;
+                rec_skip[j] = A.rec_out && !used;
                 ridx[j] = r;
-                const float tm2 = used ? A.t0[sbase + s] + A.t1[sbase + s] : 0.0f;
+                const float tm2 = used ? tsum : 0.0f;
 #pragma unroll
                 for (int a = 0; a < 3; ++a) px[j][a] = A.rays_o[3 * r + a] + (A.rays_d[3 * r + a] * tm2) / 2.0f;
                 tq[j] = A.t_per_ray ? A.timestamps[r] : A.timestamps[0];
@@ -281,12 +300,18 @@
         to_operand<4, true, NT>(D, B);
         mlp_layer<16, 1, NT>(lw + BL::B1, lane, B, D);
 
-#pragma unroll
-        for (int j = 0; j < NT; ++j) {
-            const int64_t s = tile * TILE + 16 * j + c;
+        float sg_rec[NT];
+#pragma unroll
+        for (int j = 0; j < NT; ++j) {
+            const int64_t s = tile * TILE + 16 * j + (lane_id_now() & 15);
             float sg = det_expf(D[j][0][HEAD16 ? 3 : 0] - 1.0f);
             sg = sel[j] ? sg : 0.0f;
-            if (g == 3 && s < n_eff) A.sigma[sbase + s] = sg;
+            sg_rec[j] = sg;
+            if (A.rec_out) {
+                if (!A.want_rgb && g == 3 && s < n_eff && !rec_skip[j]) A.rec_out[sbase + s].sigma = sg;
+            } else if (g == 3 && s < n_eff) {
+                A.sigma[sbase + s] = sg;
+            }
             if (A.geo && s < n_eff) {
 #pragma unroll
                 for (int r = 0; r < 4; ++r) {
@@ -328,11 +353,15 @@
 #pragma unroll
                 for (int j = 0; j < NT; ++j) {
                     const float o1 = 1.0f / (1.0f + det_expf(-D[j][0][0]));
-                    int lane_now = (int)threadIdx.x;
-                    asm volatile("" : "+v"(lane_now));
+                    const int lane_now = lane_id_now();
                     const int g_now = (lane_now >> 4) & 3;
                     const int64_t s_now = tile * TILE + 16 * j + (lane_now & 15);
-                    if (g_now < 3 && s_now < n_eff) A.rgb[3 * (sbase + s_now) + g_now] = o1;
+                    if (A.rec_out) {
+                        if (s_now < n_eff && !rec_skip[j])
+                            reinterpret_cast<float *>(A.rec_out)[4 * (sbase + s_now) + g_now] = g_now < 3 ? o1 : sg_rec[j];
+                    } else if (g_now < 3 && s_now < n_eff) {
+                        A.rgb[3 * (sbase + s_now) + g_now] = o1;
+                    }
                 }
             }
             continue;
@@ -366,15 +395,19 @@
             for (int j = 0; j < NT; ++j) {
                 const int64_t s = tile * TILE + 16 * j + c;
                 const float o1 = 1.0f / (1.0f + det_expf(-D[j][0][0]));
-                int lane_now = (int)threadIdx.x;
-                asm volatile("" : "+v"(lane_now));
+                const int lane_now = lane_id_now();
                 const int g_now = (lane_now >> 4) & 3;
                 const int64_t s_now = tile * TILE + 16 * j + (lane_now & 15);
-                if (g_now < 3 && s_now < n_eff) A.rgb[3 * (sbase + s_now) + g_now] = o1;
-            }
-        }
-    }
-    if (A.stamp && lane == 0) atomicMax(A.stamp + 1, (unsigned long long)wall_clock64());
-}
-
-}
+                if (A.rec_out) {
+                    if (s_now < n_eff && !rec_skip[j])
+                        reinterpret_cast<float *>(A.rec_out)[4 * (sbase + s_now) + g_now] = g_now < 3 ? o1 : sg_rec[j];
+                } else if (g_now < 3 && s_now < n_eff) {
+                    A.rgb[3 * (sbase + s_now) + g_now] = o1;
+                }
+            }
+        }
+    }
+    if (A.stamp && lane_id_now() == 0) atomicMax(A.stamp + 1, (unsigned long long)wall_clock64());
+}
+
+}
diff --git a/ced_nerf_amd/csrc/frame.hip b/ced_nerf_amd/csrc/frame.hip
--- a/ced_nerf_amd/csrc/frame.hip
+++ b/ced_nerf_amd/csrc/frame.hip
@@ -316,8 +316,7 @@
     const float *t_sorted;
     const uint8_t *t_indices;
     const uint8_t *hits;
-    float *t_starts, *t_ends;
-    int32_t *ray_idx;
+    SampleIn *samples;
     int32_t *packed;
     int32_t *cand;
 };
@@ -437,7 +436,7 @@
         } else {
             f = frame_of_slot(P, A.n_frames, s0);
             if (f < 0) continue;
-            const int64_t idx = s0 + threadIdx.x - P.slot_base[f];
+            const int idx = (int)(s0 - P.slot_base[f]) + (int)threadIdx.x;
             active = idx < P.count[f];
             const int64_t first = (int64_t)f * A.rays_per_frame;
             r = active ? (A.alive ? (int64_t)A.alive[first + idx] : first + idx) : 0;
@@ -471,9 +470,8 @@
         if (active) {
             A.packed[2 * r] = (int32_t)start;
             A.packed[2 * r + 1] = n;
-            float *const p0 = A.t_starts + start, *const p1 = A.t_ends + start;
-            int32_t *const pr = A.ray_idx + start;
-            const auto store = [&](int i, float t0, float t1) { p0[i] = t0; p1[i] = t1; pr[i] = (int32_t)r; };
+            SampleIn *const ps = A.samples + start;
+            const auto store = [&](int i, float t0, float t1) { ps[i] = SampleIn{ t0, t1, (int32_t)r, (int32_t)(r >> 32) }; };
             if (n > 0 && !runs.replayable(grid)) {
                 float unused;
                 (void)walk(store, unused);
@@ -520,9 +518,9 @@
 
 __global__ __launch_bounds__(kCompositeThreads) void frame_composite_kernel(
     IterPlan *plan, int n_frames, int rays_per_frame, const int32_t *__restrict__ alive_list,
-    int32_t *__restrict__ next_list, const int32_t *__restrict__ packed, const float *__restrict__ t0,
-    const float *__restrict__ t1, const float *__restrict__ sig, const float *__restrict__ rgbs, float *__restrict__ rgb,
-    float *__restrict__ opacity, float *__restrict__ depth, float opc_thres)
+    int32_t *__restrict__ next_list, const int32_t *__restrict__ packed, const SampleIn *__restrict__ rec_in,
+    const SampleOut *__restrict__ rec_out, float *__restrict__ rgb, float *__restrict__ opacity, float *__restrict__ depth,
+    float opc_thres)
 {
     const IterPlan &P = *plan;
     const int64_t total = P.total_slots;
@@ -551,8 +549,10 @@
                     float ts[kU], te[kU], sg[kU], cr[kU], cg[kU], cb[kU];
 #pragma unroll
                     for (int u = 0; u < kU; ++u) {
-                        ts[u] = t0[i + u]; te[u] = t1[i + u]; sg[u] = sig[i + u];
-                        cr[u] = rgbs[3 * (i + u)]; cg[u] = rgbs[3 * (i + u) + 1]; cb[u] = rgbs[3 * (i + u) + 2];
+                        const float2 tt = *reinterpret_cast<const float2 *>(rec_in + (i + u));
+                        const float4 o = *reinterpret_cast<const float4 *>(rec_out + (i + u));
+                        ts[u] = tt.x; te[u] = tt.y; sg[u] = o.w;
+                        cr[u] = o.x; cg[u] = o.y; cb[u] = o.z;
                     }
 #pragma unroll
                     for (int u = 0; u < kU; ++u) {
@@ -569,14 +569,16 @@
                     }
                 }
                 for (; i < end; ++i) {
-                    float ts = t0[i], te = t1[i];
-                    float sd = sig[i] * (te - ts);
+                    const float2 tt = *reinterpret_cast<const float2 *>(rec_in + i);
+                    const float4 o = *reinterpret_cast<const float4 *>(rec_out + i);
+                    float ts = tt.x, te = tt.y;
+                    float sd = o.w * (te - ts);
                     float a = 1.0f - det_expf(-sd);
                     float t = det_expf(-acc) * prefix;
                     float w = t * a;
-                    c0 = c0 + w * rgbs[3 * i];
-                    c1 = c1 + w * rgbs[3 * i + 1];
-                    c2 = c2 + w * rgbs[3 * i + 2];
+                    c0 = c0 + w * o.x;
+                    c1 = c1 + w * o.y;
+                    c2 = c2 + w * o.z;
                     op = op + w;
                     dp = dp + w * ((ts + te) / 2.0f);
                     acc = acc + sd;
@@ -912,7 +914,8 @@
     IterPlan *plans;
     float *lattice;
     float *ts_ray;
-    float *t0, *t1; int32_t *ridx; float *sigma, *rgbs;
+    SampleIn *rec_in;
+    SampleOut *rec_out;
     uint8_t *accel;
     size_t bytes;
 };
@@ -944,11 +947,8 @@
     w.plans = c.take<IterPlan>((size_t)max_iters + 2);
     w.lattice = c.take<float>(256);
     w.ts_ray = c.take<float>(per_ray_times ? (size_t)n : 0);
-    w.t0 = c.take<float>((size_t)cap);
-    w.t1 = c.take<float>((size_t)cap);
-    w.ridx = c.take<int32_t>((size_t)cap);
-    w.sigma = c.take<float>((size_t)cap);
-    w.rgbs = c.take<float>((size_t)cap * 3);
+    w.rec_in = c.take<SampleIn>((size_t)cap);
+    w.rec_out = c.take<SampleOut>((size_t)cap);
     const int64_t nbk = (res + kBrick - 1) / kBrick;
     w.accel = c.take<uint8_t>((size_t)(2 * m * nbk * nbk * nbk));
     w.bytes = c.off;
@@ -1056,6 +1056,7 @@
     CED_REQUIRE(rays_o && rays_d && binaries && aabbs && (timestamps || frame_times) && rgb && opacity && depth &&
                     workspace && host_stats,
                 "%s: null pointer", who);
+    CED_REQUIRE(((uintptr_t)workspace & 15) == 0, "%s: the workspace must be 16-byte aligned (sample records)", who);
     const int min_samples = min_samples_of(cone_angle);
     const int64_t cap = sample_capacity(n_frames, rays_per_frame, min_samples, xch ? xch->global_rays_per_frame : 0);
     CED_REQUIRE(cap < (1ll << 31) - 64, "%s: too many samples per iteration for 32-bit sample indices", who);
@@ -1118,7 +1119,7 @@
         const int64_t slot_bound = alive_bound + (int64_t)n_frames * kSlotAlign;
         MarchArgs M{ rays_o, rays_d, GridSpec{ binaries, aabbs, n_grids, res, step_size, cone_angle, 0, use_lattice ? W.lattice : nullptr },
                      acc, W.near, far_plane, cur_list, n_frames,
-                     (int)rays_per_frame, W.t_sorted, W.t_indices, W.hits, W.t0, W.t1, W.ridx, W.packed, W.alive_b };
+                     (int)rays_per_frame, W.t_sorted, W.t_indices, W.hits, W.rec_in, W.packed, W.alive_b };
         int64_t mgrid = (slot_bound + kMarchThreads - 1) / kMarchThreads;
         if (mgrid > 8192) mgrid = 8192;
         const dim3 mblk(kMarchThreads);
@@ -1148,11 +1149,11 @@
         FieldArgs F{};
         F.n = cap;
         F.n_dev = &plan->total_samples;
-        F.rays_o = rays_o; F.rays_d = rays_d; F.ray_idx32 = W.ridx;
-        F.t0 = W.t0; F.t1 = W.t1;
+        F.rays_o = rays_o; F.rays_d = rays_d;
+        F.rec_in = W.rec_in; F.rec_out = W.rec_out;
         F.timestamps = frame_times ? W.ts_ray : timestamps;
         F.rays_mode = 1; F.t_per_ray = (frame_times || t_per_ray) ? 1 : 0; F.want_rgb = 1;
-        F.rgb = W.rgbs; F.sigma = W.sigma; F.geo = nullptr;
+        F.geo = nullptr;
         if (trace && trace->field_stamps && it < trace->capacity)
             F.stamp = reinterpret_cast<unsigned long long *>(trace->field_stamps) + 2 * it;
         if (split) {
@@ -1174,7 +1175,7 @@
         if (cgrid > 4096) cgrid = 4096;
         plan_seq[it + 1] = ++g_publish_seq;
         hipLaunchKernelGGL(frame_composite_kernel, dim3((unsigned)cgrid), dim3(kCompositeThreads), 0, stream,
-                           plan, n_frames, (int)rays_per_frame, cur_list, next_list, W.packed, W.t0, W.t1, W.sigma, W.rgbs,
+                           plan, n_frames, (int)rays_per_frame, cur_list, next_list, W.packed, W.rec_in, W.rec_out,
                            rgb, opacity, depth, opc_thres);
         int64_t *xrow = nullptr;
         if (xch) {
diff --git a/ced_nerf_amd/ops.py b/ced_nerf_amd/ops.py
--- a/ced_nerf_amd/ops.py
+++ b/ced_nerf_amd/ops.py
@@ -232,6 +232,23 @@
                                                int(bool(want_rgb)), _p(rgb), _p(sigma), _stream())
     _lib.check(rc, "field_forward_rays")
     return rgb, sigma
+
+
+def field_forward_records(desc: _lib.FieldDesc, rays_o, rays_d, records_in, timestamps, t_per_ray: bool, want_rgb: bool,
+                          records_out, n_dev: Optional[torch.Tensor] = None):
+    _chk(rays_o, torch.float32, "rays_o"); _chk(rays_d, torch.float32, "rays_d")
+    _chk(records_in, torch.int32, "records_in"); _chk(records_out, torch.float32, "records_out")
+    _chk(timestamps, torch.float32, "timestamps")
+    n = records_in.shape[0]
+    assert records_in.shape == (n, 4) and records_out.shape == (n, 4)
+    if t_per_ray:
+        assert timestamps.numel() == rays_o.shape[0], "per-ray timestamps must have one entry per ray"
+    with profiling.span("field", n):
+        rc = _lib.lib().ced_field_forward_records(C.byref(desc), n, _p(n_dev), _p(rays_o), _p(rays_d), _p(records_in),
+                                                  _p(timestamps), int(bool(t_per_ray)), int(bool(want_rgb)),
+                                                  _p(records_out), _stream())
+    _lib.check(rc, "field_forward_records")
+    return records_out
 
 
 def field_move(desc: _lib.FieldDesc, positions, t, want=(True, True, True, True)):
diff --git a/include/cednerf_hip.h b/include/cednerf_hip.h
--- a/include/cednerf_hip.h
+++ b/include/cednerf_hip.h
@@ -125,6 +125,11 @@
                            const int64_t *ray_indices, const float *t_starts, const float *t_ends,
                            const float *timestamps, int32_t t_per_ray, int32_t want_rgb,
                            float *rgb, float *sigma, void *stream);
+
+int ced_field_forward_records(const ced_field_desc *desc, int64_t n, const int64_t *n_dev,
+                              const float *rays_o, const float *rays_d, const void *records_in,
+                              const float *timestamps, int32_t t_per_ray, int32_t want_rgb,
+                              void *records_out, void *stream);
 
 int ced_field_move(const ced_field_desc *desc, int64_t n, const float *positions, const float *t,
                    float *x_move, float *move, float *x_norm, uint8_t *selector, void *stream);
```

Result: no change. 4.437 billion (median of 4 runs) (+0.3%).
